# jinggqu/NextGen-UIA

Hardware: AMD Instinct MI355X
Metric: images/sec fwd+bwd BiomedCLIP+Mona bs=256 (higher is better)
Workload: dtype bf16

## Files before the change

### include/uia_hip.h

```cpp
#ifndef UIA_HIP_H
#define UIA_HIP_H
#include <stddef.h>
#include <stdint.h>

#ifdef __cplusplus
extern "C" {
#endif

enum { UIA_F32 = 0, UIA_BF16 = 1 };
enum { UIA_ACT_NONE = 0, UIA_ACT_GELU = 1, UIA_ACT_QUICKGELU = 2, UIA_ACT_RELU = 3 };
enum { UIA_MASK_NONE = 0, UIA_MASK_CAUSAL = 1, UIA_MASK_KEYPAD = 2 };
enum { UIA_MONA_BASELINE = 0, UIA_MONA_NOISE_AWARE = 1, UIA_MONA_FREQ_ENHANCED = 2, UIA_MONA_HYBRID = 3 };

const char* uia_last_error(void);
int uia_version(void);

typedef struct uia_gemm_desc {
    const void* A; int64_t lda;
    const void* W; int64_t ldw;
    int32_t M, N, K;
    float alpha;
    const float* bias;
    int32_t act;
    int32_t dact;
// ... 144 lines not shown
    const void* w1; const float* b1;
    const void* w2; const float* b2;
    float* y32;
    void* yT; int64_t yT_kb_rows;
    int64_t* rowsum_out;
    int32_t* ln_flag;
    void* u_out;
    void* t_out;
} uia_mona_fused_desc;
int uia_mona_fused_supported(int dtype, int D, int h, int w, int bott);
int uia_mona_fused_fwd(void* stream, int dtype, const uia_mona_fused_desc* d);

typedef struct uia_lora_rank_desc {
    int32_t M, N, nsrc;
    float alpha;
    const void* Q; int64_t ldq, q_stride;
    const void* W[3]; int64_t ldw;
    void* out; int64_t ldo;
    float drop_p;
    uint64_t seed[3];
} uia_lora_rank_desc;
int uia_lora_rank_update(void* stream, int dtype, const uia_lora_rank_desc* d);

typedef struct uia_ln_lora_desc {
    int32_t M, D, nsrc;
    float eps;
    const float* x; int64_t ldx;
    const float *gamma, *beta;
    void* h;
    const void* A[3]; int64_t lda;
    void* T; int64_t t_stride;
    float drop_p;
    uint64_t seed[3];
} uia_ln_lora_desc;
int uia_ln_lora_down(void* stream, int dtype, const uia_ln_lora_desc* d);

int uia_upsample_bilinear_fwd(void* stream, int B, int C, int h, int w, int H, int W, const float* src, int64_t ld, float* dst);
int uia_upsample_bilinear_bwd(void* stream, int B, int C, int h, int w, int H, int W, const float* ddst, float* dsrc, int64_t ld);
int uia_segment_mean_fwd(void* stream, int B, int n, int C, const float* x, int64_t ld, float* out);
int uia_segment_mean_bwd(void* stream, int B, int n, int C, const float* dout, float* dx, int64_t ld);
size_t uia_dicece_workspace_bytes(int B);
int uia_dicece_fwd_bwd(void* stream, int B, int C, int HW, const float* logits, const float* label, float smooth_nr, float smooth_dr,
                       float* ws, float* loss, float* dlogits);
size_t uia_focal_workspace_bytes(int N, int C);
int uia_focal_fwd_bwd(void* stream, int N, int C, const float* logits, const int64_t* labels, float gamma, float alpha, void* ws, size_t ws_bytes,
                      float* loss, float* dlogits);
size_t uia_binary_cls_stats_workspace_bytes(int N);
int uia_binary_cls_stats(void* stream, int N, const float* p1, const int64_t* labels, const int64_t* perm, void* ws, size_t ws_bytes, double* record);
size_t uia_surface_distances_workspace_bytes(int B, int H, int W);
int uia_surface_distances(void* stream, int B, int H, int W, const float* logits, const float* label, float percentile, void* ws, size_t ws_bytes,
                          double* hd, double* asd);
size_t uia_retrieval_workspace_bytes(int N, int E);
int uia_retrieval_ranks(void* stream, int N, int E, const float* img, const float* txt, int normalize, void* ws, size_t ws_bytes,
                        int32_t* gt_i2t, int32_t* eq_i2t, int32_t* gt_t2i, int32_t* eq_t2i);
size_t uia_retrieval_stats_workspace_bytes(int N);
int uia_retrieval_stats(void* stream, int N, const int32_t* gt, int nk, const int32_t* k_values, void* ws, size_t ws_bytes, double* record);

int uia_cast(void* stream, int dtype, size_t n, const float* src, void* dst, float scale);
int uia_transpose_cast(void* stream, int dtype, int rows, int cols, const float* src, void* dst);

typedef struct uia_pack_desc {
    const float* src;
    void* row;
    void* row_kb;
    void* tr;
    void* tr_kb;
    int32_t rows, cols;
    int32_t rows_pad, cols_pad;
    float scale;
    int32_t reserved_;
} uia_pack_desc;
int uia_pack_weights(void* stream, int dtype, int n, const uia_pack_desc* descs_device, int max_elems);
int uia_im2col(void* stream, int dtype, int B, int C, int H, int W, int P, const float* img, void* out);
int uia_im2col_padded(void* stream, int dtype, int B, int C, int H, int W, int P, const float* img, void* cols, int64_t ldo);
int uia_fill_cls(void* stream, int B, int N, int D, const float* cls, const float* pos0, float* x);
int uia_embed(void* stream, int rows, int L, int D, int vocab, int max_pos, const int64_t* ids, const float* table, const float* pos,
              const float* type0, float* out);
int uia_embed_packed(void* stream, int rows, int D, int vocab, int max_pos, const int64_t* ids, const int64_t* pos_idx, const float* table,
                     const float* pos, const float* type0, float* out);
int uia_embed_bwd(void* stream, int rows, int D, int vocab, const int64_t* ids, const float* dx, float* dtable, int64_t pad_id);
int uia_gather_rows(void* stream, int n, int D, const float* src, const int64_t* idx, float* dst);
int uia_copy_rows(void* stream, int rows, int64_t row_bytes, const void* src, int64_t src_stride_bytes, void* dst);
int uia_rows3_to_f32(void* stream, int rows, int D, int64_t stride_rows, const void* hi, int64_t ldhi, int64_t hi_kb_rows, const int8_t* lo, int64_t ldlo, float* dst);
int uia_dropout(void* stream, int dtype, size_t n, const void* src, void* dst, float p, uint64_t seed, int accumulate);
int uia_colsum(void* stream, int dtype, int M, int N, const void* A, int64_t lda, float* out);

int uia_layernorm_bwd_affine(void* stream, int dtype, int M, int D, const void* dy, const float* x, const float* gamma, float eps,
                             const float* dres, float* dx32, float* g_gamma, float* g_beta);
int uia_film_fwd(void* stream, int B, int N, int C, const float* x, const float* mul, const float* add, float* y);
int uia_film_bwd(void* stream, int B, int N, int C, const float* dy, const float* x, const float* mul, float* dx, float* dmul, float* dadd);
int uia_im2col3x3(void* stream, int dtype, int B, int h, int w, int C, int ntok, int tok_off, const float* x, void* cols);
int uia_col2im3x3(void* stream, int dtype, int B, int h, int w, int C, int ntok, int tok_off, const void* dcols, float* dx);
int uia_unshuffle(void* stream, int dtype, int B, int h, int w, int k1, int k2, const void* tmp, int64_t ld, float bias, float* out);
int uia_shuffle(void* stream, int dtype, int B, int h, int w, int k1, int k2, const float* dout, void* dtmp, int64_t ld);
int uia_act_bwd(void* stream, int dtype, size_t n, const void* dy, const void* y, int act, void* out);

size_t uia_infonce_workspace_bytes(int B, int E);
int uia_infonce_fwd_bwd(void* stream, int B, int E, const float* img, const float* txt, float inv_temp, float grad_scale,
                        float* loss, float* dimg, float* dtxt, void* workspace, size_t workspace_bytes);

int uia_adamw_clip_step(void* stream, size_t n, float* p, const float* g, float* m, float* v, float lr, float beta1, float beta2,
                        float eps, float weight_decay, float max_norm, int step, float grad_scale, float* ws2);

int uia_grad_accum_guarded(void* stream, size_t n, float* acc, float* mb, const float* loss, float* stats, int32_t* ctl, uint8_t* ok_log, int64_t log_index);
int uia_adamw_clip_step_guarded(void* stream, size_t n, float* p, float* acc, float* m, float* v, float lr, float lr_min, int t_max, float beta1, float beta2,
                                float eps, float weight_decay, float max_norm, float grad_scale, float skip_scale, float* ws8, int32_t* ctl);

enum { UIA_CONV3 = 0, UIA_CONVT_FWD = 1, UIA_CONVT_BWD = 2, UIA_CONV1 = 3 };
#define UIA_WGRAD_MAX_SPLITS 64
#define UIA_WGRAD_MAX_NARROW_SPLITS 512
#define UIA_WGRAD_MAX_DIRECT_SPLITS 1024
int uia_conv_igemm(void* stream, int dtype, int mode, int B, int H, int W, int C1, int C2, const void* x1, const void* x2, int N, int N1,
                   const void* w, const float* bias, void* y1, void* y2);
int uia_conv_wgrad_splits(int mode, int B, int H, int W, int C1, int C2, int N);
int uia_conv_igemm_form(int mode, int C1, int C2, int N, int N1);
int uia_conv_wgrad_form(int mode, int C1, int C2, int N);
int uia_conv_wgrad(void* stream, int dtype, int mode, int B, int H, int W, int C1, int C2, const void* x1, const void* x2, int N, const void* dy,
                   float* ws, float* dw);
#define UIA_BN_SLICES 256
int uia_bn_fwd(void* stream, int dtype, int training, int64_t M, int C, const void* y, const float* gamma, const float* beta, float* running_mean,
               float* running_var, int64_t* num_batches_tracked, float momentum, float eps, float* ws, float* mean, float* invstd, float* scale,
               float* shift, int relu, void* out);
int uia_bn_relu_bwd(void* stream, int dtype, int64_t M, int C, const void* y, const void* dout, const float* scale, const float* shift,
                    const float* mean, const float* invstd, const float* gamma, float* ws, float* dgamma, float* dbeta, void* dy);
int uia_colsum_ordered(void* stream, int dtype, int64_t M, int C, const void* y, float* ws, float* out);
int uia_bn_act_fwd(void* stream, int dtype, int training, int64_t M, int C, const void* y, const float* gamma, const float* beta, float* running_mean,
                   float* running_var, int64_t* num_batches_tracked, float momentum, float eps, float* ws, float* mean, float* invstd, float* scale,
                   float* shift, float slope, void* out, float drop_p, uint64_t seed, const uint8_t* keep_mask);
int uia_bn_act_bwd(void* stream, int dtype, int64_t M, int C, const void* y, const void* dout, const float* scale, const float* shift,
                   const float* mean, const float* invstd, const float* gamma, float* ws, float* dgamma, float* dbeta, void* dy, float slope,
                   float drop_p, uint64_t seed, const uint8_t* keep_mask);
int uia_maxpool2_fwd(void* stream, int dtype, int B, int H, int W, int C, const void* x, void* y);
int uia_maxpool2_bwd(void* stream, int dtype, int B, int H, int W, int C, const void* x, const void* dy, void* dx);
int uia_upsample_ac(void* stream, int dtype, int backward, int B, int H, int W, int C, int f, const void* in, void* out);
int uia_resize_aa(void* stream, int dtype, int backward, int B, int C, int Hi, int Wi, int Ho, int Wo, const void* x, float* tmp, float* out,
                  const float* dout, void* dx);

int uia_conv_strided(void* stream, int dtype, int dgrad, int B, int H, int W, int C, int k, int s, const void* x, int N, const void* w, void* y);
int uia_conv_strided_wgrad_splits(int B, int H, int W, int C, int k, int s, int N);
int uia_conv_strided_form(int dgrad, int C, int N, int k, int s);
int uia_conv_strided_wgrad_form(int C, int N, int k, int s);
int uia_conv_strided_wgrad(void* stream, int dtype, int B, int H, int W, int C, int k, int s, const void* x, int N, const void* dy, float* ws,
                           float* dw);
int uia_maxpool3s2_fwd(void* stream, int dtype, int B, int H, int W, int C, const void* x, void* y);
int uia_maxpool3s2_bwd(void* stream, int dtype, int B, int H, int W, int C, const void* x, const void* dy, void* dx);
int uia_bn_add_relu_fwd(void* stream, int dtype, int training, int64_t M, int C, const void* y, const void* r, const float* gamma, const float* beta,
                        float* running_mean, float* running_var, int64_t* num_batches_tracked, float momentum, float eps, float* ws, float* mean,
                        float* invstd, float* scale, float* shift, void* out);
int uia_bn_add_relu_bwd(void* stream, int dtype, int64_t M, int C, const void* y, const void* out, const void* dout, const float* mean,
                        const float* invstd, const float* gamma, float* ws, float* dgamma, float* dbeta, void* dy, void* dr);
int uia_avgpool_fwd(void* stream, int dtype, int B, int H, int W, int C, const void* x, float* pooled);
int uia_avgpool_bwd(void* stream, int dtype, int B, int H, int W, int C, const float* dout, void* dx);
int uia_nchw_to_nhwc(void* stream, int dtype, int B, int Cin, int H, int W, int Cout, int rep, const float* x, void* out);
int uia_add2(void* stream, int dtype, int64_t n, const void* a, const void* b, void* out);

int uia_comm_unique_id_bytes(void);
int uia_comm_get_unique_id(void* out, int bytes);
int uia_comm_init(int rank, int world, const void* unique_id, int bytes);
int uia_comm_world(void);
int uia_comm_initialised(void);
int uia_allreduce_sum(void* stream, int dtype, void* buf, size_t n);
int uia_allgather(void* stream, int dtype, const void* send, void* recv, size_t n_per_rank);
int uia_comm_destroy(void);

#ifdef __cplusplus
}
// ... 3 lines not shown
```

### nextgen-uia_amd/csrc/capi.cpp

```cpp
#include "uia_kernels.h"

void uia_set_error(const char* fmt, ...);
#define NEED(ptr, name) do { if (!(ptr)) { uia_set_error("%s: null descriptor", name); return -1; } } while (0)

extern "C" {

int uia_version(void) { return 100; }

int uia_gemm(void* stream, int dtype, const uia_gemm_desc* d, int tile_cfg) {
    NEED(d, "uia_gemm");
    return uia_gemm_launch((hipStream_t)stream, dtype, *d, tile_cfg);
}
int uia_lora_rank_update(void* stream, int dtype, const uia_lora_rank_desc* d) {
    NEED(d, "uia_lora_rank_update");
    return uia_lora_rank_update_launch((hipStream_t)stream, dtype, *d);
}
int uia_ln_lora_down(void* stream, int dtype, const uia_ln_lora_desc* d) {
    NEED(d, "uia_ln_lora_down");
    return uia_ln_lora_down_launch((hipStream_t)stream, dtype, *d);
}
int uia_wgrad(void* stream, int dtype, int M, int I, int J, const void* A, int64_t lda, const void* B, int64_t ldb, float alpha, float* dW, float* dbias_A) {
    return uia_wgrad_launch((hipStream_t)stream, dtype, M, I, J, A, lda, B, ldb, alpha, dW, dbias_A);
}
int uia_wgrad_ex(void* stream, int dtype, int M, int I, int J, const void* A, int64_t lda, const void* B, int64_t ldb, float alpha, float* dW, int64_t ldw,
                 int i_valid, int j_valid, float* dbias_A) {
    if (ldw <= 0) { uia_set_error("uia_wgrad_ex: ldw=%lld must be positive", (long long)ldw); return -1; }
    return uia_wgrad_launch((hipStream_t)stream, dtype, M, I, J, A, lda, B, ldb, alpha, dW, dbias_A, ldw, i_valid, j_valid);
}
int uia_wgrad_group(void* stream, int dtype, const uia_wgrad_group_desc* d) {
    if (!d) { uia_set_error("uia_wgrad_group: null descriptor"); return -1; }
    if (d->n < 1 || d->n > 4) { uia_set_error("uia_wgrad_group: n=%d outside 1..4", d->n); return -1; }
    if (d->ldw <= 0) { uia_set_error("uia_wgrad_group: ldw=%lld must be positive", (long long)d->ldw); return -1; }
    float* dW[4];
    float* db[4];
    for (int g = 0; g < 4; ++g) { dW[g] = d->dW[g]; db[g] = d->dbias_A[g]; }
    if (d->drop_p > 0.f) for (int g = 0; g < d->n; ++g) if (db[g]) { uia_set_error("uia_wgrad_group: dbias with dropout on B is not a form of the kernel"); return -1; }
    return uia_wgrad_group_launch((hipStream_t)stream, dtype, d->n, d->M, d->I, d->J, d->A, (long)d->lda, d->B, (long)d->ldb, d->alpha, dW, db, (long)d->ldw, d->i_valid, d->j_valid,
                                  d->drop_p, d->drop_seed, (long)d->drop_ld, d->drop_col0);
}
int uia_wgrad_drop(void* stream, int dtype, int M, int I, int J, const void* A, int64_t lda, const void* B, int64_t ldb, float alpha, float* dW, int64_t ldw,
                   int i_valid, int j_valid, float drop_p, uint64_t seed, int64_t drop_ld, int drop_col0) {
    if (ldw <= 0) { uia_set_error("uia_wgrad_drop: ldw=%lld must be positive", (long long)ldw); return -1; }
    if (!(drop_p > 0.f)) { uia_set_error("uia_wgrad_drop: drop_p=%f must be in (0, 1); uia_wgrad_ex is the form without dropout", (double)drop_p); return -1; }
    return uia_wgrad_launch((hipStream_t)stream, dtype, M, I, J, A, lda, B, ldb, alpha, dW, nullptr, ldw, i_valid, j_valid, drop_p, seed, drop_ld, drop_col0);
}
int uia_attn_fwd(void* stream, int dtype, const uia_attn_desc* d) {
    NEED(d, "uia_attn_fwd");
    return uia_attn_fwd_launch((hipStream_t)stream, dtype, *d);
}
int uia_attn_fwd_long(void* stream, int dtype, const uia_attn_desc* d) {
    NEED(d, "uia_attn_fwd_long");
    return uia_attn_fwd_long_launch((hipStream_t)stream, dtype, *d);
}
int uia_attn_bwd(void* stream, int dtype, const uia_attn_desc* d) {
    NEED(d, "uia_attn_bwd");
    return uia_attn_bwd_launch((hipStream_t)stream, dtype, *d, 0);
}
int uia_attn_bwd_cfg(void* stream, int dtype, const uia_attn_desc* d, int cfg) {
    NEED(d, "uia_attn_bwd_cfg");
    return uia_attn_bwd_launch((hipStream_t)stream, dtype, *d, cfg);
}
int uia_layernorm_fwd(void* stream, int dtype, int M, int D, int64_t ldx, const float* x, const float* gamma, const float* beta, float eps, void* yT, float* y32) {
    return uia_layernorm_fwd_launch((hipStream_t)stream, dtype, M, D, ldx, x, gamma, beta, eps, yT, y32, nullptr);
}
int uia_layernorm_fwd_stats(void* stream, int dtype, int M, int D, int64_t ldx, const float* x, const float* gamma, const float* beta, float eps, void* yT, float* y32,
                            float* stats) {
    return uia_layernorm_fwd_launch((hipStream_t)stream, dtype, M, D, ldx, x, gamma, beta, eps, yT, y32, stats);
}
int uia_layernorm_bwd(void* stream, int dtype, int M, int D, int64_t ldx, const void* dy, const float* x, const float* gamma, float eps, const float* dres, float* dx32, void* dxT) {
    return uia_layernorm_bwd_launch((hipStream_t)stream, dtype, M, D, ldx, dy, x, gamma, eps, dres, dx32, dxT);
}
int uia_layernorm_bwd3(void* stream, int dtype, int M, int D, int64_t ldx, const void* dy, const float* x, const void* x_hi, const int8_t* x_lo, int64_t x_kb_rows,
                       const float* gamma, float eps, const float* dres, const void* dres_hi, const int8_t* dres_lo, int64_t dres_kb_rows, float* dx32, void* dxT,
                       int8_t* dx_lo) {
    return uia_layernorm_bwd3_launch((hipStream_t)stream, dtype, M, D, ldx, dy, x, x_hi, x_lo, (long)x_kb_rows, gamma, eps, dres, dres_hi, dres_lo, (long)dres_kb_rows, dx32, dxT,
                                     dx_lo);
}
int uia_layernorm_bwd_periodic(void* stream, int dtype, int M, int D, const void* dy, const float* x, const void* x_hi, const int8_t* x_lo, int64_t x_kb_rows,
                               const float* gamma, float eps, const float* dres_rows, int period, float* dx32, void* dxT, int8_t* dx_lo) {
    return uia_layernorm_bwd_periodic_launch((hipStream_t)stream, dtype, M, D, dy, x, x_hi, x_lo, (long)x_kb_rows, gamma, eps, dres_rows, period, dx32, dxT, dx_lo);
}
int uia_attn_bwd_cls(void* stream, int dtype, const uia_attn_desc* d) {
    NEED(d, "uia_attn_bwd_cls");
    return uia_attn_bwd_cls_launch((hipStream_t)stream, dtype, *d);
}
int uia_attn_bwd_cls_rows(void* stream, int dtype, const uia_attn_desc* d) {
    NEED(d, "uia_attn_bwd_cls_rows");
    return uia_attn_bwd_cls_launch((hipStream_t)stream, dtype, *d, true);
}
int uia_attn_fwd_cls(void* stream, int dtype, const uia_attn_desc* d) {
    NEED(d, "uia_attn_fwd_cls");
    return uia_attn_fwd_cls_launch((hipStream_t)stream, dtype, *d);
}
int uia_mona_cls_fwd(void* stream, int dtype, int B, int ntok, const void* t, int64_t ldt, void* d, float p_drop, uint64_t seed, const uint8_t* keep_mask) {
    return uia_mona_cls_fwd_launch((hipStream_t)stream, dtype, B, ntok, t, (long)ldt, d, p_drop, seed, keep_mask);
}
int uia_rows3_to_f32(void* stream, int rows, int D, int64_t stride_rows, const void* hi, int64_t ldhi, int64_t hi_kb_rows, const int8_t* lo, int64_t ldlo, float* dst) {
    return uia_rows3_to_f32_launch((hipStream_t)stream, rows, D, (long)stride_rows, hi, (long)ldhi, (long)hi_kb_rows, lo, (long)ldlo, dst);
}
int uia_mona_cls_bwd(void* stream, int dtype, int B, int ntok, const void* dd, const void* t, int64_t ldt, void* dt, float p_drop, uint64_t seed, const uint8_t* keep_mask) {
    return uia_mona_cls_bwd_launch((hipStream_t)stream, dtype, B, ntok, dd, t, (long)ldt, dt, p_drop, seed, keep_mask);
}
int uia_copy_rows(void* stream, int rows, int64_t row_bytes, const void* src, int64_t src_stride_bytes, void* dst) {
    return uia_copy_rows_launch((hipStream_t)stream, rows, (long)row_bytes, src, (long)src_stride_bytes, dst);
}
int uia_cast(void* stream, int dtype, size_t n, const float* src, void* dst, float scale) { return uia_cast_launch((hipStream_t)stream, dtype, n, src, dst, scale); }
int uia_transpose_cast(void* stream, int dtype, int rows, int cols, const float* src, void* dst) { return uia_transpose_cast_launch((hipStream_t)stream, dtype, rows, cols, src, dst); }
int uia_pack_weights(void* stream, int dtype, int n, const uia_pack_desc* descs_device, int max_elems) { return uia_pack_weights_launch((hipStream_t)stream, dtype, n, descs_device, max_elems); }
int uia_im2col(void* stream, int dtype, int B, int C, int H, int W, int P, const float* img, void* out) { return uia_im2col_launch((hipStream_t)stream, dtype, B, C, H, W, P, img, out); }
int uia_fill_cls(void* stream, int B, int N, int D, const float* cls, const float* pos0, float* x) { return uia_fill_cls_launch((hipStream_t)stream, B, N, D, cls, pos0, x); }
int uia_embed(void* stream, int rows, int L, int D, int vocab, int max_pos, const int64_t* ids, const float* table, const float* pos, const float* type0, float* out) {
    return uia_embed_launch((hipStream_t)stream, rows, L, D, vocab, max_pos, ids, table, pos, type0, out);
}
int uia_gather_rows(void* stream, int n, int D, const float* src, const int64_t* idx, float* dst) { return uia_gather_rows_launch((hipStream_t)stream, n, D, src, idx, dst); }

int uia_mona_pre_fwd(void* stream, int dtype, int M, int D, const float* x, const float* norm_w, const float* norm_b, const float* gamma,
                     const float* gammax, float eps, void* u) {
    return uia_mona_pre_fwd_launch((hipStream_t)stream, dtype, M, D, x, norm_w, norm_b, gamma, gammax, eps, u);
}
int uia_mona_pre_bwd(void* stream, int dtype, int M, int D, const void* du, const float* x, const float* dy, const float* norm_w,
                     const float* norm_b, const float* gamma, const float* gammax, float eps, float* dx32, void* dxT, float* g_gamma,
                     float* g_gammax, float* g_norm_w, float* g_norm_b, float* ws, int64_t dxT_kb_rows) {
    return uia_mona_pre_bwd_launch((hipStream_t)stream, dtype, M, D, du, x, dy, norm_w, norm_b, gamma, gammax, eps, dx32, dxT, g_gamma, g_gammax,
                                   g_norm_w, g_norm_b, ws, (long)dxT_kb_rows);
}
int uia_mona_pre_fwd_t(void* stream, int dtype, int M, int D, const float* x, const float* norm_w, const float* norm_b, const float* gamma, const float* gammax,
                       float eps, void* u, const void* w1, int64_t ldw1, const float* b1, void* t, int64_t ldt) {
    return uia_mona_pre_fwd_t_launch((hipStream_t)stream, dtype, M, D, x, norm_w, norm_b, gamma, gammax, eps, u, w1, (long)ldw1, b1, t, (long)ldt);
}
int uia_mona_pre_bwd_du(void* stream, int dtype, int M, int D, const void* dt, int64_t ldt, const void* w1t, int64_t ldw1, const float* x, const float* dy,
                        const float* norm_w, const float* norm_b, const float* gamma, const float* gammax, float eps, float* dx32, void* dxT, float* g_gamma,
                        float* g_gammax, float* g_norm_w, float* g_norm_b, float* ws, int64_t dxT_kb_rows) {
    if (!dt || !w1t) { uia_set_error("uia_mona_pre_bwd_du: null dt / w1t"); return -1; }
    return uia_mona_pre_bwd_launch((hipStream_t)stream, dtype, M, D, nullptr, x, dy, norm_w, norm_b, gamma, gammax, eps, dx32, dxT, g_gamma, g_gammax,
                                   g_norm_w, g_norm_b, ws, (long)dxT_kb_rows, dt, (long)ldt, w1t, (long)ldw1);
}
int uia_mona_pre_bwd_du3(void* stream, int dtype, int M, int D, const void* dt, int64_t ldt, const void* w1t, int64_t ldw1, const float* x, const void* dy_hi, const int8_t* dy_lo,
                         const float* norm_w, const float* norm_b, const float* gamma, const float* gammax, float eps, void* dxT, int8_t* dx_lo, float* g_gamma,
                         float* g_gammax, float* g_norm_w, float* g_norm_b, float* ws, int64_t dxT_kb_rows) {
    if (!dt || !w1t || !dy_hi || !dy_lo || !dx_lo) { uia_set_error("uia_mona_pre_bwd_du3: null dt / w1t / dy_hi / dy_lo / dx_lo"); return -1; }
    return uia_mona_pre_bwd_launch((hipStream_t)stream, dtype, M, D, nullptr, x, nullptr, norm_w, norm_b, gamma, gammax, eps, nullptr, dxT, g_gamma, g_gammax,
                                   g_norm_w, g_norm_b, ws, (long)dxT_kb_rows, dt, (long)ldt, w1t, (long)ldw1, dy_hi, dy_lo, dx_lo);
}
size_t uia_mona_pre_bwd_workspace_bytes(int M, int D) { return uia_mona_pre_bwd_ws_floats(M, D) * sizeof(float); }
int uia_mona_spatial_fwd(void* stream, int dtype, const uia_mona_spatial_desc* d) {
    NEED(d, "uia_mona_spatial_fwd");
    return uia_mona_spatial_fwd_launch((hipStream_t)stream, dtype, *d);
}
int uia_mona_spatial_bwd(void* stream, int dtype, const uia_mona_spatial_desc* d) {
    NEED(d, "uia_mona_spatial_bwd");
    return uia_mona_spatial_bwd_launch((hipStream_t)stream, dtype, *d);
}
int uia_mona_fused_fwd(void* stream, int dtype, const uia_mona_fused_desc* d) {
    NEED(d, "uia_mona_fused_fwd");
    return uia_mona_fused_fwd_launch((hipStream_t)stream, dtype, *d);
}

size_t uia_infonce_workspace_bytes(int B, int E) { return uia_infonce_workspace_floats(B, E) * sizeof(float); }
int uia_infonce_fwd_bwd(void* stream, int B, int E, const float* img, const float* txt, float inv_temp, float grad_scale, float* loss,
                        float* dimg, float* dtxt, void* workspace, size_t workspace_bytes) {
    return uia_infonce_launch((hipStream_t)stream, B, E, img, txt, inv_temp, grad_scale, loss, dimg, dtxt, (float*)workspace, workspace_bytes / sizeof(float));
}
int uia_adamw_clip_step(void* stream, size_t n, float* p, const float* g, float* m, float* v, float lr, float beta1, float beta2, float eps,
                        float weight_decay, float max_norm, int step, float grad_scale, float* ws2) {
    return uia_adamw_clip_launch((hipStream_t)stream, n, p, g, m, v, lr, beta1, beta2, eps, weight_decay, max_norm, step, grad_scale, ws2);
}
int uia_grad_accum_guarded(void* stream, size_t n, float* acc, float* mb, const float* loss, float* stats, int32_t* ctl, uint8_t* ok_log, int64_t log_index) {
    return uia_grad_accum_guarded_launch((hipStream_t)stream, n, acc, mb, loss, stats, (int*)ctl, ok_log, (long)log_index);
}
int uia_adamw_clip_step_guarded(void* stream, size_t n, float* p, float* acc, float* m, float* v, float lr, float lr_min, int t_max, float beta1, float beta2,
                                float eps, float weight_decay, float max_norm, float grad_scale, float skip_scale, float* ws8, int32_t* ctl) {
    return uia_adamw_clip_guarded_launch((hipStream_t)stream, n, p, acc, m, v, lr, lr_min, t_max, beta1, beta2, eps, weight_decay, max_norm, grad_scale, skip_scale, ws8, (int*)ctl);
}

int uia_dropout(void* stream, int dtype, size_t n, const void* src, void* dst, float p, uint64_t seed, int accumulate) {
    return uia_dropout_launch((hipStream_t)stream, dtype, n, src, dst, p, seed, accumulate);
}
int uia_colsum(void* stream, int dtype, int M, int N, const void* A, int64_t lda, float* out) {
    return uia_colsum_launch((hipStream_t)stream, dtype, M, N, A, lda, out);
}

int uia_layernorm_bwd_affine(void* stream, int dtype, int M, int D, const void* dy, const float* x, const float* gamma, float eps, const float* dres,
                             float* dx32, float* g_gamma, float* g_beta) {
    return uia_layernorm_bwd_affine_launch((hipStream_t)stream, dtype, M, D, dy, x, gamma, eps, dres, dx32, g_gamma, g_beta);
}
int uia_film_fwd(void* stream, int B, int N, int C, const float* x, const float* mul, const float* add, float* y) { return uia_film_fwd_launch((hipStream_t)stream, B, N, C, x, mul, add, y); }
int uia_film_bwd(void* stream, int B, int N, int C, const float* dy, const float* x, const float* mul, float* dx, float* dmul, float* dadd) {
    return uia_film_bwd_launch((hipStream_t)stream, B, N, C, dy, x, mul, dx, dmul, dadd);
// ... 165 lines not shown
```

### nextgen-uia_amd/csrc/uia_kernels.h

```cpp
#pragma once
#include <hip/hip_runtime.h>
#include <stddef.h>
#include <stdint.h>

#include "../../include/uia_hip.h"

typedef uia_gemm_desc UiaGemmParams;
typedef uia_attn_desc UiaAttnParams;

int uia_gemm_launch(hipStream_t stream, int dtype, const UiaGemmParams& p, int cfg);
int uia_attn_fwd_launch(hipStream_t stream, int dtype, const UiaAttnParams& p);
int uia_attn_fwd_long_launch(hipStream_t stream, int dtype, const UiaAttnParams& p);
int uia_attn_bwd_launch(hipStream_t stream, int dtype, const UiaAttnParams& p, int cfg = 0);
int uia_layernorm_fwd_launch(hipStream_t stream, int dtype, int M, int D, long ldx, const float* x, const float* gamma, const float* beta,
                             float eps, void* yT, float* y32, float* stats);
int uia_layernorm_bwd_launch(hipStream_t stream, int dtype, int M, int D, long ldx, const void* dy, const float* x, const float* gamma, float eps,
                             const float* dres, float* dx32, void* dxT);
int uia_layernorm_bwd3_launch(hipStream_t stream, int dtype, int M, int D, long ldx, const void* dy, const float* x, const void* x_hi, const int8_t* x_lo,
                              long x_kb_rows, const float* gamma, float eps, const float* dres, const void* dres_hi, const int8_t* dres_lo, long dres_kb_rows,
                              float* dx32, void* dxT, int8_t* dx_lo);
int uia_layernorm_bwd_periodic_launch(hipStream_t stream, int dtype, int M, int D, const void* dy, const float* x, const void* x_hi, const int8_t* x_lo, long x_kb_rows,
                                      const float* gamma, float eps, const float* dres_rows, int period, float* dx32, void* dxT, int8_t* dx_lo);
int uia_attn_bwd_cls_launch(hipStream_t stream, int dtype, const UiaAttnParams& p, bool compact = false);
int uia_attn_fwd_cls_launch(hipStream_t stream, int dtype, const UiaAttnParams& p);
int uia_mona_cls_fwd_launch(hipStream_t stream, int dtype, int B, int ntok, const void* t, long ldt, void* d, float p_drop, uint64_t seed, const uint8_t* keep_mask);
int uia_rows3_to_f32_launch(hipStream_t stream, int rows, int D, long stride_rows, const void* hi, long ldhi, long hi_kb_rows, const int8_t* lo, long ldlo, float* dst);
int uia_mona_cls_bwd_launch(hipStream_t stream, int dtype, int B, int ntok, const void* dd, const void* t, long ldt, void* dt, float p_drop, uint64_t seed,
                            const uint8_t* keep_mask);
int uia_copy_rows_launch(hipStream_t stream, int rows, long row_bytes, const void* src, long src_stride_bytes, void* dst);
int uia_lora_rank_update_launch(hipStream_t stream, int dtype, const uia_lora_rank_desc& p);
int uia_ln_lora_down_launch(hipStream_t stream, int dtype, const uia_ln_lora_desc& p);
int uia_cast_launch(hipStream_t stream, int dtype, size_t n, const float* src, void* dst, float scale);
int uia_transpose_cast_launch(hipStream_t stream, int dtype, int rows, int cols, const float* src, void* dst);
int uia_pack_weights_launch(hipStream_t stream, int dtype, int n, const uia_pack_desc* descs_device, int max_elems);
int uia_im2col_launch(hipStream_t stream, int dtype, int B, int C, int H, int W, int P, const float* img, void* out);
int uia_fill_cls_launch(hipStream_t stream, int B, int N, int D, const float* cls, const float* pos0, float* x);
int uia_embed_launch(hipStream_t stream, int rows, int L, int D, int vocab, int max_pos, const int64_t* ids, const float* table, const float* pos, const float* type0, float* out);
int uia_gather_rows_launch(hipStream_t stream, int n, int D, const float* src, const int64_t* idx, float* dst);
int uia_wgrad_group_launch(hipStream_t stream, int dtype, int n, int M, int I, int J, const void* const* A, long lda, const void* const* B, long ldb, float alpha,
                            float* const* dW, float* const* dbias, long ldw, int i_valid, int j_valid, float drop_p, const uint64_t* drop_seed, long drop_ld, int drop_col0);
int uia_wgrad_launch(hipStream_t stream, int dtype, int M, int I, int J, const void* A, long lda, const void* B, long ldb, float alpha, float* dW, float* dbias,
                     long ldw = 0, int i_valid = 0, int j_valid = 0, float drop_p = 0.f, uint64_t drop_seed = 0, long drop_ld = 0, int drop_col0 = 0);
int uia_mona_pre_fwd_launch(hipStream_t stream, int dtype, int M, int D, const float* x, const float* nw, const float* nb, const float* gamma,
                            const float* gammax, float eps, void* u);
int uia_mona_pre_fwd_t_launch(hipStream_t stream, int dtype, int M, int D, const float* x, const float* nw, const float* nb, const float* gamma,
                              const float* gammax, float eps, void* u, const void* w1, long ldw1, const float* b1, void* t, long ldt);
int uia_mona_pre_bwd_launch(hipStream_t stream, int dtype, int M, int D, const void* du, const float* x, const float* dy, const float* nw,
                            const float* nb, const float* gamma, const float* gammax, float eps, float* dx32, void* dxT, float* g_gamma,
                            float* g_gammax, float* g_nw, float* g_nb, float* ws, long dxT_kb_rows, const void* dt = nullptr, long ldt = 0,
                            const void* w1t = nullptr, long ldw1 = 0, const void* dy_hi = nullptr, const int8_t* dy_lo = nullptr, int8_t* dx_lo = nullptr);
size_t uia_mona_pre_bwd_ws_floats(int M, int D);
int uia_mona_spatial_fwd_launch(hipStream_t stream, int dtype, const uia_mona_spatial_desc& p);
int uia_mona_spatial_bwd_launch(hipStream_t stream, int dtype, const uia_mona_spatial_desc& p);
int uia_mona_fused_fwd_launch(hipStream_t stream, int dtype, const uia_mona_fused_desc& q);
size_t uia_infonce_workspace_floats(int B, int E);
int uia_infonce_launch(hipStream_t stream, int B, int E, const float* img, const float* txt, float inv_temp, float grad_scale, float* loss,
                       float* dimg, float* dtxt, float* ws, size_t ws_floats);
int uia_adamw_clip_launch(hipStream_t stream, size_t n, float* p, const float* g, float* m, float* v, float lr, float beta1, float beta2,
                          float eps, float weight_decay, float max_norm, int step, float grad_scale, float* ws);
int uia_grad_accum_guarded_launch(hipStream_t stream, size_t n, float* acc, float* mb, const float* loss, float* stats, int* ctl, unsigned char* ok_log, long log_index);
int uia_adamw_clip_guarded_launch(hipStream_t stream, size_t n, float* p, float* acc, float* m, float* v, float lr, float lr_min, int t_max, float beta1,
                                  float beta2, float eps, float weight_decay, float max_norm, float grad_scale, float skip_scale, float* ws8, int* ctl);
int uia_dropout_launch(hipStream_t stream, int dtype, size_t n, const void* src, void* dst, float p, uint64_t seed, int accumulate);
int uia_colsum_launch(hipStream_t stream, int dtype, int M, int N, const void* A, long lda, float* out);
int uia_attn_small_launch(hipStream_t stream, int dtype, const UiaAttnParams& p, bool bwd);
bool uia_attn_dh16_ok(int dtype, const UiaAttnParams& p);
int uia_attn_dh16_launch(hipStream_t stream, const UiaAttnParams& p, bool bwd);
int uia_layernorm_bwd_affine_launch(hipStream_t stream, int dtype, int M, int D, const void* dy, const float* x, const float* gamma, float eps,
                                    const float* dres, float* dx32, float* g_gamma, float* g_beta);
int uia_film_fwd_launch(hipStream_t stream, int B, int N, int C, const float* x, const float* mul, const float* add, float* y);
int uia_film_bwd_launch(hipStream_t stream, int B, int N, int C, const float* dy, const float* x, const float* mul, float* dx, float* dmul, float* dadd);
int uia_im2col3x3_launch(hipStream_t stream, int dtype, int B, int h, int w, int C, int ntok, int tok_off, const float* x, void* cols);
int uia_col2im3x3_launch(hipStream_t stream, int dtype, int B, int h, int w, int C, int ntok, int tok_off, const void* dcols, float* dx);
int uia_unshuffle_launch(hipStream_t stream, int dtype, int B, int h, int w, int k1, int k2, const void* tmp, long ld, float bias, float* out);
int uia_shuffle_launch(hipStream_t stream, int dtype, int B, int h, int w, int k1, int k2, const float* dout, void* dtmp, long ld);
int uia_act_bwd_launch(hipStream_t stream, int dtype, size_t n, const void* dy, const void* y, int act, void* out);
size_t uia_mona_spatial_ws_floats(int B);
int uia_upsample_bilinear_launch(hipStream_t stream, bool bwd, int B, int C, int h, int w, int H, int W, const float* in, float* out, long ld);
int uia_segment_mean_launch(hipStream_t stream, bool bwd, int B, int n, int C, const float* in, float* out, long ld);
size_t uia_dicece_ws_floats(int B);
int uia_dicece_launch(hipStream_t stream, int B, int C, int HW, const float* logits, const float* label, float nr, float dr, float* ws, float* loss, float* dlogits);
size_t uia_focal_ws_bytes(int N, int C);
int uia_focal_launch(hipStream_t stream, int N, int C, const float* logits, const int64_t* labels, float gamma, float alpha, void* ws, size_t ws_bytes,
                     float* loss, float* dlogits);
size_t uia_binary_cls_stats_ws_bytes(int N);
int uia_binary_cls_stats_launch(hipStream_t stream, int N, const float* p1, const int64_t* labels, const int64_t* perm, void* ws, size_t ws_bytes,
                                double* record);
size_t uia_surface_ws_bytes(int B, int H, int W);
int uia_surface_launch(hipStream_t stream, int B, int H, int W, const float* logits, const float* label, float percentile, void* ws, size_t ws_bytes,
                       double* hd, double* asd);
size_t uia_retrieval_ranks_ws_bytes(int N, int E);
int uia_retrieval_ranks_launch(hipStream_t stream, int N, int E, const float* img, const float* txt, int normalize, void* ws, size_t ws_bytes,
                               int32_t* gt_i2t, int32_t* eq_i2t, int32_t* gt_t2i, int32_t* eq_t2i);
size_t uia_retrieval_stats_ws_bytes(int N);
int uia_retrieval_stats_launch(hipStream_t stream, int N, const int32_t* gt, int nk, const int32_t* k_values, void* ws, size_t ws_bytes, double* record);
int uia_im2col_padded_launch(hipStream_t stream, int dtype, int B, int C, int H, int W, int P, const float* img, void* out, long ldo);
int uia_embed_bwd_launch(hipStream_t stream, int rows, int D, int vocab, const int64_t* ids, const float* dx, float* dtable, long pad_id);
int uia_embed_packed_launch(hipStream_t stream, int rows, int D, int vocab, int max_pos, const int64_t* ids, const int64_t* pos_idx, const float* table, const float* pos, const float* type0, float* out);
int uia_ln_mean_rows_launch(hipStream_t stream, int B, int L, int row0, int n, int D, long ldx, const float* x, const float* gamma, const float* beta,
                            float eps, float* ws, float* out, long ldo);
int uia_conv_igemm_launch(hipStream_t stream, int dtype, int mode, int B, int H, int W, int C1, int C2, const void* x1, const void* x2, int N, int N1,
                          const void* w, const float* bias, void* y1, void* y2);
int uia_conv_wgrad_splits(int mode, int B, int H, int W, int C1, int C2, int N);
int uia_conv_wgrad_launch(hipStream_t stream, int dtype, int mode, int B, int H, int W, int C1, int C2, const void* x1, const void* x2, int N,
                          const void* dy, float* ws, float* dw);
int uia_bn_fwd_launch(hipStream_t stream, int dtype, int training, long M, int C, const void* y, const float* gamma, const float* beta,
                      float* run_mean, float* run_var, int64_t* nbt, float momentum, float eps, float* ws, float* mean, float* invstd,
                      float* scale, float* shift, int relu, void* out);
int uia_bn_relu_bwd_launch(hipStream_t stream, int dtype, long M, int C, const void* y, const void* dout, const float* scale, const float* shift,
                           const float* mean, const float* invstd, const float* gamma, float* ws, float* dgamma, float* dbeta, void* dy);
int uia_colsum_ordered_launch(hipStream_t stream, int dtype, long M, int C, const void* y, float* ws, float* out);
int uia_conv_igemm_form(int mode, int C1, int C2, int N, int N1);
// ... 28 lines not shown
```

### nextgen-uia_amd/uia_hip/_lib.py

```python
import ctypes as C
import os
import re

import torch

_HERE = os.path.dirname(os.path.abspath(__file__))
LIB_PATH = os.environ.get("UIA_HIP_LIB") or os.path.join(_HERE, "libuia_hip.so")

F32, BF16 = 0, 1
ACT_NONE, ACT_GELU, ACT_QUICKGELU, ACT_RELU = 0, 1, 2, 3
MASK_NONE, MASK_CAUSAL, MASK_KEYPAD = 0, 1, 2
MONA_VARIANTS = {"baseline": 0, "noise_aware": 1, "freq_enhanced": 2, "hybrid": 3}

vp, i32, i64, f32, sz = C.c_void_p, C.c_int32, C.c_int64, C.c_float, C.c_size_t


class PackDesc(C.Structure):
    _fields_ = [("src", vp), ("row", vp), ("row_kb", vp), ("tr", vp), ("tr_kb", vp), ("rows", i32), ("cols", i32),
                ("rows_pad", i32), ("cols_pad", i32), ("scale", f32), ("reserved_", i32)]


class GemmDesc(C.Structure):
    _fields_ = [("A", vp), ("lda", i64), ("W", vp), ("ldw", i64), ("M", i32), ("N", i32), ("K", i32), ("alpha", f32),
                ("bias", vp), ("act", i32), ("dact", i32), ("aux_in", vp), ("ldaux_in", i64), ("aux_out", vp), ("ldaux_out", i64),
                ("resid", vp), ("ldr", i64), ("resid_mod", i32), ("resid_row_off", i32), ("residT", vp), ("ldrT", i64),
                ("out_group", i32), ("outT", vp), ("ldo", i64), ("out32", vp), ("ldo32", i64), ("w_kblocked", i32),
                ("resid_ln_stats", vp), ("resid_ln_w", vp), ("resid_ln_b", vp),
                ("rowsum_out", vp), ("lnfold_sums", vp), ("lnfold_colsum", vp), ("lnfold_dim", i32), ("lnfold_eps", f32),
                ("resid_ln_dim", i32), ("resid_ln_eps", f32), ("a_kb_rows", i64), ("outT_kb_rows", i64), ("ln_flag", vp), ("ln_flag_limit", f32),
                ("drop_where", i32), ("drop_p", f32), ("drop_seed", C.c_uint64), ("a_drop_out", vp), ("splitk_ws", vp),
                ("A2", vp), ("lda2", i64), ("K2", i32), ("a2_group_cols", i32), ("a2_group_stride", i64),
                ("resid_lo8", vp), ("ld_resid_lo", i64), ("residT_kb_rows", i64), ("out_lo8", vp), ("ld_out_lo", i64),
                ("resid_lo_kb_rows", i64), ("out_lo_kb_rows", i64)]


class AttnDesc(C.Structure):
    _fields_ = [("q", vp), ("k", vp), ("v", vp), ("ld_qkv", i64), ("out", vp), ("ldo", i64), ("lse", vp), ("keylen", vp),
                ("B", i32), ("H", i32), ("L", i32), ("dh", i32), ("mask_kind", i32), ("scale", f32),
                ("dout", vp), ("lddo", i64), ("dq", vp), ("dk", vp), ("dv", vp), ("ld_dqkv", i64), ("cu_seqlens", vp),
                ("out_kb_rows", i64), ("dqkv_kb_rows", i64)]


class MonaSpatialDesc(C.Structure):
    _fields_ = [("variant", i32), ("B", i32), ("h", i32), ("w", i32), ("bott", i32),
                ("t", vp), ("d", vp),
                ("conv1_w", vp), ("conv1_b", vp), ("conv2_w", vp), ("conv2_b", vp), ("conv3_w", vp), ("conv3_b", vp),
                ("proj_w", vp), ("proj_b", vp), ("freq", vp), ("ne1_w", vp), ("ne1_b", vp), ("ne3_w", vp), ("ne3_b", vp),
                ("p_drop", f32), ("seed", C.c_uint64), ("keep_mask", vp),
                ("dd", vp), ("dt", vp),
                ("g_conv1_w", vp), ("g_conv1_b", vp), ("g_conv2_w", vp), ("g_conv2_b", vp), ("g_conv3_w", vp), ("g_conv3_b", vp),
                ("g_proj_w", vp), ("g_proj_b", vp), ("g_freq", vp), ("g_ne1_w", vp), ("g_ne1_b", vp), ("g_ne3_w", vp), ("g_ne3_b", vp), ("ws", vp)]


class WgradGroupDesc(C.Structure):
    _fields_ = [("n", C.c_int32), ("M", C.c_int32), ("I", C.c_int32), ("J", C.c_int32), ("A", C.c_void_p * 4), ("B", C.c_void_p * 4), ("dW", C.c_void_p * 4),
                ("dbias_A", C.c_void_p * 4), ("lda", C.c_int64), ("ldb", C.c_int64), ("ldw", C.c_int64), ("i_valid", C.c_int32), ("j_valid", C.c_int32),
                ("alpha", C.c_float), ("drop_p", C.c_float), ("drop_seed", C.c_uint64 * 4), ("drop_ld", C.c_int64), ("drop_col0", C.c_int32), ("reserved", C.c_int32)]


class LoraRankDesc(C.Structure):
    _fields_ = [("M", i32), ("N", i32), ("nsrc", i32), ("alpha", f32), ("Q", vp), ("ldq", i64), ("q_stride", i64), ("W", vp * 3), ("ldw", i64),
                ("out", vp), ("ldo", i64), ("drop_p", f32), ("seed", C.c_uint64 * 3)]


class LnLoraDesc(C.Structure):
    _fields_ = [("M", i32), ("D", i32), ("nsrc", i32), ("eps", f32), ("x", vp), ("ldx", i64), ("gamma", vp), ("beta", vp), ("h", vp), ("A", vp * 3), ("lda", i64),
                ("T", vp), ("t_stride", i64), ("drop_p", f32), ("seed", C.c_uint64 * 3)]


class MonaFusedDesc(C.Structure):
    _fields_ = [("sp", MonaSpatialDesc), ("D", i32), ("eps", f32), ("x", vp), ("norm_w", vp), ("norm_b", vp), ("gamma", vp), ("gammax", vp),
                ("w1", vp), ("b1", vp), ("w2", vp), ("b2", vp), ("y32", vp), ("yT", vp), ("yT_kb_rows", i64), ("rowsum_out", vp), ("ln_flag", vp),
                ("u_out", vp), ("t_out", vp)]


PROTOTYPES = {
    "uia_last_error": (C.c_char_p, []),
    "uia_version": (C.c_int, []),
    "uia_gemm": (C.c_int, [vp, C.c_int, C.POINTER(GemmDesc), C.c_int]),
    "uia_wgrad": (C.c_int, [vp, C.c_int, C.c_int, C.c_int, C.c_int, vp, i64, vp, i64, f32, vp, vp]),
    "uia_wgrad_drop": (C.c_int, [vp, C.c_int, C.c_int, C.c_int, C.c_int, vp, i64, vp, i64, f32, vp, i64, C.c_int, C.c_int, f32, C.c_uint64, i64, C.c_int]),
    "uia_wgrad_group": (C.c_int, [vp, C.c_int, vp]),
    "uia_wgrad_ex": (C.c_int, [vp, C.c_int, C.c_int, C.c_int, C.c_int, vp, i64, vp, i64, f32, vp, i64, C.c_int, C.c_int, vp]),
    "uia_attn_fwd": (C.c_int, [vp, C.c_int, C.POINTER(AttnDesc)]),
    "uia_attn_fwd_long": (C.c_int, [vp, C.c_int, C.POINTER(AttnDesc)]),
    "uia_attn_bwd": (C.c_int, [vp, C.c_int, C.POINTER(AttnDesc)]),
    "uia_attn_bwd_cfg": (C.c_int, [vp, C.c_int, C.POINTER(AttnDesc), C.c_int]),
    "uia_layernorm_fwd": (C.c_int, [vp, C.c_int, C.c_int, C.c_int, i64, vp, vp, vp, f32, vp, vp]),
    "uia_layernorm_fwd_stats": (C.c_int, [vp, C.c_int, C.c_int, C.c_int, i64, vp, vp, vp, f32, vp, vp, vp]),
    "uia_ln_mean_rows": (C.c_int, [vp, C.c_int, C.c_int, C.c_int, C.c_int, C.c_int, i64, vp, vp, vp, f32, vp, vp, i64]),
    "uia_conv_igemm": (C.c_int, [vp, C.c_int, C.c_int, C.c_int, C.c_int, C.c_int, C.c_int, C.c_int, vp, vp, C.c_int, C.c_int, vp, vp, vp, vp]),
    "uia_conv_wgrad_splits": (C.c_int, [C.c_int, C.c_int, C.c_int, C.c_int, C.c_int, C.c_int, C.c_int]),
    "uia_conv_wgrad": (C.c_int, [vp, C.c_int, C.c_int, C.c_int, C.c_int, C.c_int, C.c_int, C.c_int, vp, vp, C.c_int, vp, vp, vp]),
    "uia_conv_igemm_form": (C.c_int, [C.c_int, C.c_int, C.c_int, C.c_int, C.c_int]),
    "uia_conv_wgrad_form": (C.c_int, [C.c_int, C.c_int, C.c_int, C.c_int]),
    "uia_bn_act_fwd": (C.c_int, [vp, C.c_int, C.c_int, i64, C.c_int, vp, vp, vp, vp, vp, vp, f32, f32, vp, vp, vp, vp, vp, f32, vp, f32, C.c_uint64, vp]),
    "uia_bn_act_bwd": (C.c_int, [vp, C.c_int, i64, C.c_int, vp, vp, vp, vp, vp, vp, vp, vp, vp, vp, vp, f32, f32, C.c_uint64, vp]),
    "uia_maxpool2_fwd": (C.c_int, [vp, C.c_int, C.c_int, C.c_int, C.c_int, C.c_int, vp, vp]),
    "uia_maxpool2_bwd": (C.c_int, [vp, C.c_int, C.c_int, C.c_int, C.c_int, C.c_int, vp, vp, vp]),
    "uia_conv_strided": (C.c_int, [vp, C.c_int, C.c_int, C.c_int, C.c_int, C.c_int, C.c_int, C.c_int, C.c_int, vp, C.c_int, vp, vp]),
    "uia_conv_strided_wgrad_splits": (C.c_int, [C.c_int, C.c_int, C.c_int, C.c_int, C.c_int, C.c_int, C.c_int]),
    "uia_conv_strided_form": (C.c_int, [C.c_int, C.c_int, C.c_int, C.c_int, C.c_int]),
    "uia_conv_strided_wgrad_form": (C.c_int, [C.c_int, C.c_int, C.c_int, C.c_int]),
    "uia_conv_strided_wgrad": (C.c_int, [vp, C.c_int, C.c_int, C.c_int, C.c_int, C.c_int, C.c_int, C.c_int, vp, C.c_int, vp, vp, vp]),
    "uia_maxpool3s2_fwd": (C.c_int, [vp, C.c_int, C.c_int, C.c_int, C.c_int, C.c_int, vp, vp]),
    "uia_maxpool3s2_bwd": (C.c_int, [vp, C.c_int, C.c_int, C.c_int, C.c_int, C.c_int, vp, vp, vp]),
    "uia_bn_add_relu_fwd": (C.c_int, [vp, C.c_int, C.c_int, i64, C.c_int, vp, vp, vp, vp, vp, vp, vp, f32, f32, vp, vp, vp, vp, vp, vp]),
    "uia_bn_add_relu_bwd": (C.c_int, [vp, C.c_int, i64, C.c_int, vp, vp, vp, vp, vp, vp, vp, vp, vp, vp, vp]),
    "uia_avgpool_fwd": (C.c_int, [vp, C.c_int, C.c_int, C.c_int, C.c_int, C.c_int, vp, vp]),
    "uia_avgpool_bwd": (C.c_int, [vp, C.c_int, C.c_int, C.c_int, C.c_int, C.c_int, vp, vp]),
    "uia_nchw_to_nhwc": (C.c_int, [vp, C.c_int, C.c_int, C.c_int, C.c_int, C.c_int, C.c_int, C.c_int, vp, vp]),
    "uia_add2": (C.c_int, [vp, C.c_int, i64, vp, vp, vp]),
    "uia_bn_fwd": (C.c_int, [vp, C.c_int, C.c_int, i64, C.c_int, vp, vp, vp, vp, vp, vp, f32, f32, vp, vp, vp, vp, vp, C.c_int, vp]),
    "uia_bn_relu_bwd": (C.c_int, [vp, C.c_int, i64, C.c_int, vp, vp, vp, vp, vp, vp, vp, vp, vp, vp, vp]),
    "uia_colsum_ordered": (C.c_int, [vp, C.c_int, i64, C.c_int, vp, vp, vp]),
    "uia_upsample_ac": (C.c_int, [vp, C.c_int, C.c_int, C.c_int, C.c_int, C.c_int, C.c_int, C.c_int, vp, vp]),
    "uia_resize_aa": (C.c_int, [vp, C.c_int, C.c_int, C.c_int, C.c_int, C.c_int, C.c_int, C.c_int, C.c_int, vp, vp, vp, vp, vp]),
    "uia_layernorm_bwd": (C.c_int, [vp, C.c_int, C.c_int, C.c_int, i64, vp, vp, vp, f32, vp, vp, vp]),
    "uia_ln_lora_down": (C.c_int, [vp, C.c_int, C.POINTER(LnLoraDesc)]),
    "uia_lora_rank_update": (C.c_int, [vp, C.c_int, C.POINTER(LoraRankDesc)]),
    "uia_layernorm_bwd3": (C.c_int, [vp, C.c_int, C.c_int, C.c_int, i64, vp, vp, vp, vp, i64, vp, f32, vp, vp, vp, i64, vp, vp, vp]),
    "uia_mona_pre_fwd": (C.c_int, [vp, C.c_int, C.c_int, C.c_int, vp, vp, vp, vp, vp, f32, vp]),
    "uia_mona_pre_bwd": (C.c_int, [vp, C.c_int, C.c_int, C.c_int, vp, vp, vp, vp, vp, vp, vp, f32, vp, vp, vp, vp, vp, vp, vp, i64]),
    "uia_mona_pre_fwd_t": (C.c_int, [vp, C.c_int, C.c_int, C.c_int, vp, vp, vp, vp, vp, f32, vp, vp, i64, vp, vp, i64]),
    "uia_mona_pre_bwd_du": (C.c_int, [vp, C.c_int, C.c_int, C.c_int, vp, i64, vp, i64, vp, vp, vp, vp, vp, vp, f32, vp, vp, vp, vp, vp, vp, vp, i64]),
    "uia_mona_pre_bwd_du3": (C.c_int, [vp, C.c_int, C.c_int, C.c_int, vp, i64, vp, i64, vp, vp, vp, vp, vp, vp, vp, f32, vp, vp, vp, vp, vp, vp, vp, i64]),
    "uia_mona_pre_bwd_workspace_bytes": (sz, [C.c_int, C.c_int]),
    "uia_mona_spatial_fwd": (C.c_int, [vp, C.c_int, C.POINTER(MonaSpatialDesc)]),
    "uia_mona_spatial_bwd": (C.c_int, [vp, C.c_int, C.POINTER(MonaSpatialDesc)]),
    "uia_mona_spatial_workspace_bytes": (sz, [C.c_int]),
    "uia_mona_fused_supported": (C.c_int, [C.c_int, C.c_int, C.c_int, C.c_int, C.c_int]),
    "uia_mona_fused_fwd": (C.c_int, [vp, C.c_int, C.POINTER(MonaFusedDesc)]),
    "uia_upsample_bilinear_fwd": (C.c_int, [vp, C.c_int, C.c_int, C.c_int, C.c_int, C.c_int, C.c_int, vp, C.c_int64, vp]),
    "uia_upsample_bilinear_bwd": (C.c_int, [vp, C.c_int, C.c_int, C.c_int, C.c_int, C.c_int, C.c_int, vp, vp, C.c_int64]),
    "uia_segment_mean_fwd": (C.c_int, [vp, C.c_int, C.c_int, C.c_int, vp, C.c_int64, vp]),
    "uia_segment_mean_bwd": (C.c_int, [vp, C.c_int, C.c_int, C.c_int, vp, vp, C.c_int64]),
    "uia_dicece_workspace_bytes": (sz, [C.c_int]),
    "uia_dicece_fwd_bwd": (C.c_int, [vp, C.c_int, C.c_int, C.c_int, vp, vp, C.c_float, C.c_float, vp, vp, vp]),
    "uia_focal_workspace_bytes": (sz, [C.c_int, C.c_int]),
    "uia_focal_fwd_bwd": (C.c_int, [vp, C.c_int, C.c_int, vp, vp, f32, f32, vp, sz, vp, vp]),
    "uia_binary_cls_stats_workspace_bytes": (sz, [C.c_int]),
    "uia_binary_cls_stats": (C.c_int, [vp, C.c_int, vp, vp, vp, vp, sz, vp]),
    "uia_surface_distances_workspace_bytes": (sz, [C.c_int, C.c_int, C.c_int]),
    "uia_surface_distances": (C.c_int, [vp, C.c_int, C.c_int, C.c_int, vp, vp, f32, vp, sz, vp, vp]),
    "uia_retrieval_workspace_bytes": (sz, [C.c_int, C.c_int]),
    "uia_retrieval_ranks": (C.c_int, [vp, C.c_int, C.c_int, vp, vp, C.c_int, vp, sz, vp, vp, vp, vp]),
    "uia_retrieval_stats_workspace_bytes": (sz, [C.c_int]),
    "uia_retrieval_stats": (C.c_int, [vp, C.c_int, vp, C.c_int, vp, vp, sz, vp]),
    "uia_infonce_workspace_bytes": (sz, [C.c_int, C.c_int]),
    "uia_infonce_fwd_bwd": (C.c_int, [vp, C.c_int, C.c_int, vp, vp, f32, f32, vp, vp, vp, vp, sz]),
    "uia_adamw_clip_step": (C.c_int, [vp, sz, vp, vp, vp, vp, f32, f32, f32, f32, f32, f32, C.c_int, f32, vp]),
    "uia_grad_accum_guarded": (C.c_int, [vp, sz, vp, vp, vp, vp, vp, vp, i64]),
    "uia_adamw_clip_step_guarded": (C.c_int, [vp, sz, vp, vp, vp, vp, f32, f32, C.c_int, f32, f32, f32, f32, f32, f32, f32, vp, vp]),
    "uia_comm_unique_id_bytes": (C.c_int, []),
    "uia_comm_get_unique_id": (C.c_int, [vp, C.c_int]),
    "uia_comm_init": (C.c_int, [C.c_int, C.c_int, vp, C.c_int]),
    "uia_comm_world": (C.c_int, []),
    "uia_comm_initialised": (C.c_int, []),
    "uia_allreduce_sum": (C.c_int, [vp, C.c_int, vp, sz]),
    "uia_allgather": (C.c_int, [vp, C.c_int, vp, vp, sz]),
    "uia_comm_destroy": (C.c_int, []),
    "uia_dropout": (C.c_int, [vp, C.c_int, sz, vp, vp, f32, C.c_uint64, C.c_int]),
    "uia_colsum": (C.c_int, [vp, C.c_int, C.c_int, C.c_int, vp, i64, vp]),
    "uia_layernorm_bwd_affine": (C.c_int, [vp, C.c_int, C.c_int, C.c_int, vp, vp, vp, f32, vp, vp, vp, vp]),
    "uia_film_fwd": (C.c_int, [vp, C.c_int, C.c_int, C.c_int, vp, vp, vp, vp]),
    "uia_film_bwd": (C.c_int, [vp, C.c_int, C.c_int, C.c_int, vp, vp, vp, vp, vp, vp]),
    "uia_im2col3x3": (C.c_int, [vp, C.c_int, C.c_int, C.c_int, C.c_int, C.c_int, C.c_int, C.c_int, vp, vp]),
    "uia_col2im3x3": (C.c_int, [vp, C.c_int, C.c_int, C.c_int, C.c_int, C.c_int, C.c_int, C.c_int, vp, vp]),
    "uia_unshuffle": (C.c_int, [vp, C.c_int, C.c_int, C.c_int, C.c_int, C.c_int, C.c_int, vp, i64, f32, vp]),
    "uia_shuffle": (C.c_int, [vp, C.c_int, C.c_int, C.c_int, C.c_int, C.c_int, C.c_int, vp, vp, i64]),
    "uia_act_bwd": (C.c_int, [vp, C.c_int, sz, vp, vp, C.c_int, vp]),
    "uia_cast": (C.c_int, [vp, C.c_int, sz, vp, vp, f32]),
    "uia_transpose_cast": (C.c_int, [vp, C.c_int, C.c_int, C.c_int, vp, vp]),
    "uia_pack_weights": (C.c_int, [vp, C.c_int, C.c_int, vp, C.c_int]),
    "uia_im2col": (C.c_int, [vp, C.c_int, C.c_int, C.c_int, C.c_int, C.c_int, C.c_int, vp, vp]),
    "uia_im2col_padded": (C.c_int, [vp, C.c_int, C.c_int, C.c_int, C.c_int, C.c_int, C.c_int, vp, vp, C.c_int64]),
    "uia_fill_cls": (C.c_int, [vp, C.c_int, C.c_int, C.c_int, vp, vp, vp]),
    "uia_embed": (C.c_int, [vp, C.c_int, C.c_int, C.c_int, C.c_int, C.c_int, vp, vp, vp, vp, vp]),
    "uia_embed_bwd": (C.c_int, [vp, C.c_int, C.c_int, C.c_int, vp, vp, vp, C.c_int64]),
    "uia_embed_packed": (C.c_int, [vp, C.c_int, C.c_int, C.c_int, C.c_int, vp, vp, vp, vp, vp, vp]),
    "uia_gather_rows": (C.c_int, [vp, C.c_int, C.c_int, vp, vp, vp]),
    "uia_copy_rows": (C.c_int, [vp, C.c_int, i64, vp, i64, vp]),
    "uia_attn_bwd_cls": (C.c_int, [vp, C.c_int, C.POINTER(AttnDesc)]),
    "uia_mona_cls_bwd": (C.c_int, [vp, C.c_int, C.c_int, C.c_int, vp, vp, i64, vp, f32, C.c_uint64, vp]),
    "uia_attn_fwd_cls": (C.c_int, [vp, C.c_int, C.POINTER(AttnDesc)]),
    "uia_attn_bwd_cls_rows": (C.c_int, [vp, C.c_int, C.POINTER(AttnDesc)]),
    "uia_mona_cls_fwd": (C.c_int, [vp, C.c_int, C.c_int, C.c_int, vp, i64, vp, f32, C.c_uint64, vp]),
    "uia_rows3_to_f32": (C.c_int, [vp, C.c_int, C.c_int, i64, vp, i64, i64, vp, i64, vp]),
    "uia_layernorm_bwd_periodic": (C.c_int, [vp, C.c_int, C.c_int, C.c_int, vp, vp, vp, vp, i64, vp, f32, vp, C.c_int, vp, vp, vp]),
}

_lib = None
_BLOCKING = ("uia_comm_init", "uia_comm_destroy", "uia_comm_get_unique_id")


class UiaError(RuntimeError):
    pass


def lib():
    global _lib
    if _lib is None:
        if not os.path.exists(LIB_PATH):
            raise UiaError(f"{LIB_PATH} not built: run `make -C nextgen-uia_amd/csrc` (hipcc --offload-arch=gfx950). "
                           "There is no CPU fallback for the uia hot path.")
        release = os.environ.get("UIA_CTYPES_RELEASE_GIL", "0") == "1"
        handle = (C.CDLL if release else C.PyDLL)(LIB_PATH)
        blocking = C.CDLL(LIB_PATH)
        _one_copy_of("librccl")
        _one_copy_of("libamdhip64")
        for name, (res, args) in PROTOTYPES.items():
            fn = getattr(blocking if name in _BLOCKING else handle, name)
            fn.restype, fn.argtypes = res, args
            if name in _BLOCKING:
                setattr(handle, name, fn)
        _lib = handle
    return _lib


def _one_copy_of(stem):
    try:
        pat = re.compile(r"^" + re.escape(stem) + r"\.so(\.\d+)*$")
        paths = {line.split()[-1] for line in open("/proc/self/maps") if pat.match(os.path.basename(line.split()[-1]) if line.split() else "")}
    except OSError:
        return
    real = {os.path.realpath(p) for p in paths}
    if len(real) > 1:
        raise UiaError(f"two copies of {stem} are loaded ({sorted(real)}): import torch before uia_hip so that libuia_hip.so binds to PyTorch's runtime")


def check(rc, what=""):
    if rc != 0:
        raise UiaError(f"{what} failed (rc={rc}): {lib().uia_last_error().decode()}")
```

### nextgen-uia_amd/uia_hip/functional.py

```python
import math
import os
import weakref

import time

import torch

from . import handoff, ops
from ._lib import UiaError
from .handoff import (ClsGrad, Resid3, _g3_partner_feeds, cls_grad_of, fwd3_of, grad3_decode, grad3_of, grad_resid3_enabled, hook_free, linear_chain,
                      publish_cls_grad, publish_fwd3, publish_grad3, publish_rows, publish_t_copy, set_cls_grad, set_grad_resid3, t_copy_of, take_rows, zero_sums,
                      cls_only, set_cls_forward, take_cls_forward)
from .handoff import clear as clear_t_copies

_STATE = {"dtype": torch.bfloat16, "seed": 0x5EED, "calls": 0, "fwd_resid3": os.environ.get("UIA_FWD_RESID3", "1") != "0"}


def set_compute_dtype(dt):
    assert dt in (torch.bfloat16, torch.float32)
    _STATE["dtype"] = dt


def compute_dtype():
    return _STATE["dtype"]
# ... 141 lines not shown
        self._table = None

    def _refreshed(self, items):
        ready = ops.Ready()
        for it in items:
            it.fwd.refreshed(ready)
            it.bwd.refreshed(ready)
            for view, _, _, _ in it.extra:
                ext = self._ext_of.get(view.untyped_storage().data_ptr())
                ext = ext() if ext is not None else None
                if ext is not None:
                    ext.ready = ready

    def _repack(self, items):
        dt, dev = items[0].dt, items[0].row.device
        entries = [e for it in items for e in it.entries()]
        table, n, mx = ops.pack_table(entries, dev)
        ops.pack_weights(table, n, mx, dt)
        for it in items:
            it.version, it.epoch, it.src_ptr = it.ref()._version, self.epoch, it.ref().data_ptr()
        self._refreshed(items)
        return table, n, mx, dt, entries

    def bump(self):
        self.epoch += 1
        if len(self._c) > 8192:
            alive = lambda r: all(x() is not None for x in r) if isinstance(r, tuple) else r() is not None
            self._c = {k: v for k, v in self._c.items() if alive(v[1])}
        live = [it for it in self._packed.values() if it.ref() is not None]
        if len(live) != len(self._packed):
            self._packed = {id(it.ref()): it for it in live}
            self._table = None
        if not live:
            return
        groups = {}
        for it in live:
            groups.setdefault((it.dt, it.row.device), []).append(it)
        tables = self._table if isinstance(self._table, dict) else {}
        fresh = {}
        for key, items in groups.items():
            sig = (sum(1 + len(it.extra) for it in items), tuple(id(it) for it in items))
            hit = tables.get(key)
            if hit is not None and hit[5] == sig and all(it.src_ptr == it.ref().data_ptr() for it in items):
                table, n, mx, dt, _, _ = hit
                ops.pack_weights(table, n, mx, dt)
                for it in items:
                    it.version, it.epoch = it.ref()._version, self.epoch
                self._refreshed(items)
                fresh[key] = hit
            else:
                fresh[key] = self._repack(items) + (sig,)
        self._table = fresh

    def _packed_get(self, p, dt, transpose, pads=None):
        it = self._packed.get(id(p))
        want = tuple(pads) if pads is not None else tuple(p.shape)
        if it is None or it.ref() is not p or it.dt != dt or it.row.device != p.device or tuple(it.row.shape) != want or it.pads != pads:
            old = it
            it = _PackedParam(p, dt, pads)
            if old is not None and old.ref() is p and old.dt == dt and old.row.device == p.device:
                it.extra = [e for e in old.extra if (self._ext_of.get(e[0].untyped_storage().data_ptr()) or (lambda: None))() is not None]
            self._packed[id(p)] = it
            self._table = None
        if it.version != p._version or it.epoch != self.epoch:
            self._repack([it])
        return it.bwd if transpose else it.fwd

    def get_lnfold(self, w, b, ln_w, ln_b, dt):
        key = (id(w), id(ln_w), dt, "lnfold")
        vers = (w._version, ln_w._version, ln_b._version, -1 if b is None else b._version, w.device)
        hit = self._c.get(key)
        if hit is not None and hit[0] == vers and hit[1]() is w and hit[3]() is ln_w:
            return hit[2]
        with torch.no_grad():
            w32 = w.detach().float()
            wf = (w32 * ln_w.detach().float()[None, :]).to(dt).contiguous()
            colsum = wf.float().sum(1).contiguous()
            bias = (w32 @ ln_b.detach().float())
            if b is not None:
                bias = bias + b.detach().float()
            bias = bias.contiguous()
        out = (ops.PackedW(wf), colsum, bias)
        self._c[key] = (vers, weakref.ref(w), out, weakref.ref(ln_w))
        return out

    def get_cat(self, ws, dt, transpose=False):
        key = (tuple(id(w) for w in ws), dt, transpose, "cat")
        vers = tuple(w._version for w in ws)
        hit = self._c.get(key)
        if hit is not None and hit[0] == vers and all(r() is w for r, w in zip(hit[1], ws)) and hit[2].device == ws[0].device:
            return hit[2]
        with torch.no_grad():
            cat = torch.cat([w.detach().float() for w in ws], 0)
            src = cat.t().contiguous() if transpose else cat
            out = ops.PackedW(src.to(dt).contiguous())
        self._c[key] = (vers, tuple(weakref.ref(w) for w in ws), out)
        return out

    def get_lora_ext(self, ws, Bs, scaling, dt, rp=64):
        key = (tuple(id(w) for w in ws), tuple(id(b) for b in Bs), dt, float(scaling), "ext")
        vers = tuple(w._version for w in ws)
        hit = self._c.get(key)
        pads = [(b.shape[0], max(rp, b.shape[1])) for b in Bs]
        if hit is not None and hit[0] == vers and all(r() is t for r, t in zip(hit[1], tuple(ws) + tuple(Bs))) and hit[2].device == ws[0].device:
            for b, pd in zip(Bs, pads):
                self._packed_get(b, dt, False, pd)
            return hit[2]
        g = 64 // torch.empty(0, dtype=dt).element_size()
        Ntot, K = sum(w.shape[0] for w in ws), ws[0].shape[1]
        assert K % g == 0 and rp % g == 0 and all(w.shape[1] == K for w in ws) and all(b.shape[0] == w.shape[0] for b, w in zip(Bs, ws))
        with torch.no_grad():
            kb = torch.zeros((K + rp) // g, Ntot, g, device=ws[0].device, dtype=dt)
            kb[:K // g] = torch.cat([w.detach().float() for w in ws], 0).to(dt).view(Ntot, K // g, g).permute(1, 0, 2)
        off = 0
        for b, pd in zip(Bs, pads):
            self._packed_get(b, dt, False, pd)
            it = self._packed[id(b)]
            it.extra = [e for e in it.extra if e[0].untyped_storage().data_ptr() != kb.untyped_storage().data_ptr()]
            it.extra.append((kb[K // g:, off:off + b.shape[0], :], Ntot, rp, float(scaling)))
            self._table = None
            self._repack([it])
            off += b.shape[0]
        out = ops.ExtW(kb, Ntot, K + rp, rp)
        self._ext_of = {k: r for k, r in self._ext_of.items() if r() is not None}
        self._ext_of[kb.untyped_storage().data_ptr()] = weakref.ref(out)
        self._c[key] = (vers, tuple(weakref.ref(t) for t in tuple(ws) + tuple(Bs)), out)
        return out

    def get(self, p, dt, transpose=False, pad_rows_to=None, pad_cols_to=None):
        padded = pad_rows_to is not None or pad_cols_to is not None
        if (p.requires_grad and (dt != torch.float32 or padded) and p.dim() == 2 and p.is_cuda
                and p.dtype == torch.float32 and p.is_contiguous() and 0 < p.numel() <= self.PACK_MAX_ELEMS):
            pads = (max(p.shape[0], pad_rows_to or 0), max(p.shape[1], pad_cols_to or 0)) if padded else None
            return self._packed_get(p, dt, transpose, pads)
        key = (id(p), dt, transpose, pad_rows_to, pad_cols_to)
        hit = self._c.get(key)
        if hit is not None and hit[0] == p._version and hit[1]() is p and hit[2].device == p.device and (not p.requires_grad or hit[3] == self.epoch):
            return hit[2]
        src = p.detach()
        if src.dim() != 2:
            src = src.reshape(src.shape[0], -1)
        src = src.contiguous().float()
        if pad_rows_to is not None and src.shape[0] < pad_rows_to:
            src = torch.cat([src, src.new_zeros(pad_rows_to - src.shape[0], src.shape[1])], 0)
        if pad_cols_to is not None and src.shape[1] < pad_cols_to:
            src = torch.cat([src, src.new_zeros(src.shape[0], pad_cols_to - src.shape[1])], 1)
        if transpose:
            out = torch.empty(src.shape[1], src.shape[0], device=src.device, dtype=dt)
            ops.transpose_cast(src, out)
        elif dt == torch.float32:
            out = src
        else:
            out = torch.empty(src.shape, device=src.device, dtype=dt)
            ops.cast(src, out)
        out = ops.PackedW(out)
        self._c[key] = (p._version, weakref.ref(p), out, self.epoch)
        return out


WEIGHTS = WeightCache()


def _empty(shape, dt, like):
    return torch.empty(shape, device=like.device, dtype=dt)


# ... 168 lines not shown
        G = ({k: p.grad for k, p in zip(names, ctx.direct_params)} if direct
             else {k: torch.zeros_like(v, dtype=torch.float32) for k, v in P.items()})
        w2t = WEIGHTS.get(P["project2.weight"], dt, transpose=True)
        dd = _empty((M, bott), dt, x)
        side = _wgrad_side_stream(x.device) if _STATE.get("wgrad_side_stream", False) else None
        _wgrad_beside(side, lambda: ops.gemm(dy_t, w2t, out_t=dd), dy_t, d, G["project2.weight"], G["project2.bias"])
        sp = {_SPATIAL_MAP[k]: v.detach().contiguous() for k, v in P.items() if k in _SPATIAL_MAP}
        sg = {_SPATIAL_MAP[k]: G[k] for k in P if k in _SPATIAL_MAP}
        dtt = _empty((M, bott), dt, x)
        ops.mona_spatial_bwd(variant, B, h, w, t, sp, dd, dtt, sg, p_drop=p_drop, seed=seed, keep_mask=keep_mask)
        w1t = WEIGHTS.get(P["project1.weight"], dt, transpose=True)
        du = None if fuse_du else _empty((M, D), dt, x)
        _wgrad_beside(side, None if fuse_du else (lambda: ops.gemm(dtt, w1t, out_t=du)), dtt, u, G["project1.weight"], G["project1.bias"])
        need_dx = ctx.needs_input_grad[0]
        dx_t = _act(M, D, dt, x, 4 * D) if (need_dx and dt != torch.float32) else None
        w1t_rows = (dtt, w1t.row if isinstance(w1t, ops.PackedW) else w1t) if fuse_du else None
        if need_dx and g3 is not None and fuse_du and getattr(ctx, "g3_out", False):
            dlo = torch.empty(M, D, device=x.device, dtype=torch.int8)
            ops.mona_pre_bwd(None, x, g3, P["norm.weight"], P["norm.bias"], P["gamma"], P["gammax"], None, dx_t,
                             G["gamma"], G["gammax"], G["norm.weight"], G["norm.bias"], dt_w1t=w1t_rows, dx_lo=dlo)
            dx = publish_grad3(x.shape, x.device, dx_t, dlo)
        else:
            if need_dx and g3 is not None:
                dy = g3.decode().view(B, N, D)
            dx = torch.empty_like(x) if need_dx else None
            ops.mona_pre_bwd(du, x, dy if need_dx else None, P["norm.weight"], P["norm.bias"], P["gamma"], P["gammax"], dx, dx_t,
                             G["gamma"], G["gammax"], G["norm.weight"], G["norm.bias"], dt_w1t=w1t_rows)
            if need_dx:
                publish_t_copy(dx, dx_t)
        grads = tuple(None if direct else (G[k] if ctx.needs_input_grad[7 + i] else None) for i, k in enumerate(names))
        return (dx, None, None, None, None, None, None) + grads


def _wgrad_beside(side, dgrad, a, b, dw, db):
    if side is not None:
        side.wait_stream(torch.cuda.current_stream())
        with torch.cuda.stream(side):
            ops.wgrad(a, b, dw, db)
        a.record_stream(side)
        b.record_stream(side)
    if dgrad is not None:
        dgrad()
    if side is None:
        ops.wgrad(a, b, dw, db)


_WGRAD_SIDE = {}


def _wgrad_side_stream(device):
    key = device.index if device.index is not None else torch.cuda.current_device()
    if key not in _WGRAD_SIDE:
        _WGRAD_SIDE[key] = torch.cuda.Stream(device=device)
    return _WGRAD_SIDE[key]


def set_wgrad_side_stream(flag):
    _STATE["wgrad_side_stream"] = bool(flag)


def join_side_streams():
    cur = torch.cuda.current_stream()
    for st in _WGRAD_SIDE.values():
        cur.wait_stream(st)


DIRECT_TRAIN = True


def _is_flat_grad(p):
    g = p.grad
    return (getattr(p, "_uia_flat_grad", False) and g is not None and g.dtype == torch.float32 and g.is_contiguous() and g.shape == p.shape
            and g.device == p.device)


def mona_apply(x_bnd, module_params, variant, hw, p_drop, training, keep_mask=None):
    names = tuple(k for k in MONA_PARAM_ORDER if k in module_params)
    pd = p_drop if (training or keep_mask is not None) else 0.0
    params = [module_params[k] for k in names]
    direct = torch.is_grad_enabled() and all(p.requires_grad and _is_flat_grad(p) for p in params)
    return MonaFn.apply(x_bnd, variant, tuple(hw), pd, keep_mask, names, direct, *params)


class BlockSpec:

    def __init__(self, heads, eps, act, ln1, qkv, proj, ln2, fc1, fc2, mask=None, publish_out=False):
        self.heads, self.eps, self.act, self.mask = heads, eps, act, mask
        self.publish_out = publish_out
        self.ln1, self.qkv, self.proj, self.ln2, self.fc1, self.fc2 = ln1, qkv, proj, ln2, fc1, fc2


ATTN_SINGLE_PASS_MAX = 272


class VitBlockFn(torch.autograd.Function):

    @staticmethod
    def forward(ctx, x, spec):
        B, N, D = x.shape
        M, dt = B * N, compute_dtype()
        if N > ATTN_SINGLE_PASS_MAX and (ctx.needs_input_grad[0] or spec.mask is not None):
            raise UiaError(f"vit_block: {N} tokens exceed the {ATTN_SINGLE_PASS_MAX} of the attention backward; sequences this long run forward-only "
                           "(frozen tower under torch.no_grad()), unmasked" if ctx.needs_input_grad[0] else
                           f"vit_block: {N} tokens with a mask: the long attention forward takes no mask")
        x3 = fwd3_of(x)
        like = x3.lo if x3 is not None else x
        if x3 is None:
            x = x.contiguous()
            x2d = x.view(M, D)
        train = ctx.needs_input_grad[0]
        fold = ln_fold_enabled(dt, M)
        if x3 is not None:
            assert fold and dt == torch.bfloat16, "a three-byte forward token reached a block that cannot take it"
            rows = (x3.hi, x3.sums)
        else:
            rows = take_rows(x, dt) if fold else None
        qkv = _empty((M, 3 * D), dt, like)
        if rows is not None:
            wq, cq, bq = WEIGHTS.get_lnfold(spec.qkv[0], spec.qkv[1], spec.ln1[0], spec.ln1[1], dt)
            xin_t, sums0 = rows
            if not ops.is_kb(xin_t):
                xin_t = xin_t.view(M, D)
            ops.gemm(xin_t, wq, bias=bq, out_t=qkv, lnfold=(sums0, cq, D, spec.eps))
            h1 = _act(M, D, dt, like, spec.fc1[0].shape[0]) if x3 is not None else xin_t
        else:
            h1 = _empty((M, D), dt, x)
            ops.layernorm_fwd(x2d, spec.ln1[0], spec.ln1[1], spec.eps, y_t=h1)
            ops.gemm(h1, WEIGHTS.get(spec.qkv[0], dt), bias=spec.qkv[1], out_t=qkv)
        if handoff.take_last_block_cls() and spec.mask is None and 1 < N <= ATTN_SINGLE_PASS_MAX and D == 64 * spec.heads and like.is_cuda:
            return VitBlockFn._forward_cls(ctx, x, x3, qkv, spec, (B, N, D), dt, train)
        if N > ATTN_SINGLE_PASS_MAX:
            a = _empty((M, D), dt, like)
            ops.attn_fwd_long(qkv[:, :D], qkv[:, D:2 * D], qkv[:, 2 * D:], a, B, spec.heads, N)
            lse = None
        else:
            a = _attn_act(M, D, dt, like, D) if D == 64 * spec.heads else _empty((M, D), dt, like)
            lse = torch.empty(B, spec.heads, N, device=like.device, dtype=torch.float32) if train else None
            ops.attn_fwd(qkv[:, :D], qkv[:, D:2 * D], qkv[:, 2 * D:], a, B, spec.heads, N, lse=lse, mask=spec.mask)
        F = spec.fc1[0].shape[0]
        f = _act(M, F, dt, like, D)
        pre = _empty((M, F), dt, like) if train else None
        r3 = fold and _STATE.get("block_resid3", False) and dt == torch.bfloat16 and M > 2048
        x1 = None if r3 else torch.empty(M, D, device=like.device, dtype=torch.float32)
        lo1 = torch.empty(M, D, device=like.device, dtype=torch.int8) if r3 else None
        if fold:
            sums1 = zero_sums(M, like.device)
            h1 = _as_act(h1, M, D, dt, F) if x3 is None else h1
            resx = dict(resid3=x3.resid3) if x3 is not None else dict(resid=x2d)
            ops.gemm(a, WEIGHTS.get(spec.proj[0], dt), bias=spec.proj[1], out32=x1, out_t=h1, out_lo=lo1, rowsum=sums1, **resx)
            w1, c1, b1 = WEIGHTS.get_lnfold(spec.fc1[0], spec.fc1[1], spec.ln2[0], spec.ln2[1], dt)
            ops.gemm(h1, w1, bias=b1, act=spec.act, aux_out=pre, out_t=f, lnfold=(sums1, c1, D, spec.eps))
        else:
            ops.gemm(a, WEIGHTS.get(spec.proj[0], dt), bias=spec.proj[1], resid=x2d, out32=x1)
            h1 = _as_act(h1, M, D, dt, 0)
            ops.layernorm_fwd(x1, spec.ln2[0], spec.ln2[1], spec.eps, y_t=h1)
            ops.gemm(h1, WEIGHTS.get(spec.fc1[0], dt), bias=spec.fc1[1], act=spec.act, aux_out=pre, out_t=f)
        x2 = torch.empty(B, N, D, device=like.device, dtype=torch.float32)
        res1 = dict(resid3=Resid3(h1, lo1)) if r3 else dict(resid=x1)
        if fold and spec.publish_out:
            sums2 = zero_sums(M, like.device)
            h2 = _act(M, D, dt, like, 3 * D) if r3 else _as_act(h1, M, D, dt, 3 * D)
            ops.gemm(f, WEIGHTS.get(spec.fc2[0], dt), bias=spec.fc2[1], out32=x2.view(M, D), out_t=h2, rowsum=sums2, **res1)
            publish_rows(x2, h2, sums2)
        else:
            ops.gemm(f, WEIGHTS.get(spec.fc2[0], dt), bias=spec.fc2[1], out32=x2.view(M, D), **res1)
        if train:
            saved, ctx.layout = handoff.save_layout(x3.resid3 if x3 is not None else x, qkv, a, lse, Resid3(h1, lo1) if r3 else x1, pre)
            ctx.save_for_backward(*saved)
            ctx.xshape = (B, N, D)
            ctx.spec = spec
            ctx.g3_out = dt == torch.bfloat16 and _g3_partner_feeds(x)
            ctx.cls_ok = spec.mask is None and N <= ATTN_SINGLE_PASS_MAX and D == 64 * spec.heads and not r3 and handoff.cls_grad_enabled()
        return x2

    @staticmethod
    def _forward_cls(ctx, x, x3, qkv, spec, shape, dt, train):
        B, N, D = shape
        like = qkv
        a = _empty((B, D), dt, like)
        lse = torch.empty(B, spec.heads, device=like.device, dtype=torch.float32) if train else None
        ops.attn_fwd_cls(qkv[:, :D], qkv[:, D:2 * D], qkv[:, 2 * D:], a, B, spec.heads, N, lse=lse)
        x_cls = torch.empty(B, D, device=like.device, dtype=torch.float32)
        if x3 is not None:
            ops.rows3_to_f32(x3.hi, x3.lo, N, x_cls)
        else:
            ops.copy_rows(x.view(B * N, D), N, x_cls)
        x1 = torch.empty(B, D, device=like.device, dtype=torch.float32)
        M = B * N
        wp = WEIGHTS.get(spec.proj[0], dt)
        ops.gemm(a, wp, bias=spec.proj[1], resid=x_cls, out32=x1, tile_cfg=_rows_tile_cfg(M, wp, like, dt, out32=True, resid=True))
        h2 = _empty((B, D), dt, like)
        ops.layernorm_fwd(x1, spec.ln2[0], spec.ln2[1], spec.eps, y_t=h2)
        F = spec.fc1[0].shape[0]
        f = _empty((B, F), dt, like)
        pre = _empty((B, F), dt, like) if train else None
        w1, w2 = WEIGHTS.get(spec.fc1[0], dt), WEIGHTS.get(spec.fc2[0], dt)
        ops.gemm(h2, w1, bias=spec.fc1[1], act=spec.act, aux_out=pre, out_t=f, tile_cfg=_rows_tile_cfg(M, w1, like, dt, act=True, aux_out=train, out_t=True))
        x2 = torch.empty(B, 1, D, device=like.device, dtype=torch.float32)
        ops.gemm(f, w2, bias=spec.fc2[1], resid=x1, out32=x2.view(B, D), tile_cfg=_rows_tile_cfg(M, w2, like, dt, out32=True, resid=True))
        if train:
            saved, ctx.layout = handoff.save_layout(x3.resid3 if x3 is not None else x, qkv, a, lse, x1, pre)
            ctx.save_for_backward(*saved)
            ctx.xshape = (B, N, D)
            ctx.spec = spec
            ctx.g3_out = dt == torch.bfloat16 and _g3_partner_feeds(x)
            ctx.cls_ok = False
            ctx.cls_fwd = True
        handoff.cls_rows_out(True)
        return x2

    @staticmethod
    def backward_cls(ctx, cg):
        compact = getattr(ctx, "cls_fwd", False)
        xin, qkv, a, lse, x1, pre = handoff.restore_layout(ctx.saved_tensors, ctx.layout)
        x3_in = isinstance(xin, Resid3)
        x = xin.lo if x3_in else xin
        spec = ctx.spec
        B, N, D = ctx.xshape
        M, dt = B * N, qkv.dtype
        F = pre.shape[1]
        dy = cg.rows32
        dy_t = dy if dt == torch.float32 else (cg.rows_t if cg.rows_t is not None else t_copy_of(dy, dt))
        pre_cls = pre if compact else ops.copy_rows(pre, N, _empty((B, F), dt, x))
        dpre = _empty((B, F), dt, x)
        ops.gemm(dy_t, WEIGHTS.get(spec.fc2[0], dt, transpose=True), dact=spec.act, aux_in=pre_cls, out_t=dpre)
        dh = _empty((B, D), dt, x)
        ops.gemm(dpre, WEIGHTS.get(spec.fc1[0], dt, transpose=True), out_t=dh)
        x1_cls = x1 if compact else ops.copy_rows(x1, N, _empty((B, D), torch.float32, x))
        dx1 = _empty((B, D), torch.float32, x)
        dx1_t = _empty((B, D), dt, x) if dt != torch.float32 else dx1
        ops.layernorm_bwd(dh, x1_cls, spec.ln2[0], spec.eps, dres=dy, dx32=dx1, dx_t=dx1_t if dt != torch.float32 else None)
        da = dh
        ops.gemm(dx1_t, WEIGHTS.get(spec.proj[0], dt, transpose=True), out_t=da)
        dqkv = _attn_act(M, 3 * D, dt, x, D)
        if ops.is_kb(dqkv):
            ops.attn_bwd_cls(qkv[:, :D], qkv[:, D:2 * D], qkv[:, 2 * D:], a, da, lse, dqkv, None, None, B, spec.heads, N, rows=compact)
        else:
            ops.attn_bwd_cls(qkv[:, :D], qkv[:, D:2 * D], qkv[:, 2 * D:], a, da, lse, dqkv[:, :D], dqkv[:, D:2 * D], dqkv[:, 2 * D:], B, spec.heads, N, rows=compact)
        dh1 = _empty((M, D), dt, x)
        ops.gemm(dqkv, WEIGHTS.get(spec.qkv[0], dt, transpose=True), out_t=dh1)
        xrows = xin if x3_in else x.view(M, D)
        if getattr(ctx, "g3_out", False):
            dx_t = _empty((M, D), dt, x)
            dlo = torch.empty(M, D, device=x.device, dtype=torch.int8)
            ops.layernorm_bwd_periodic(dh1, xrows, spec.ln1[0], spec.eps, dx1, N, dx_t=dx_t, dx_lo=dlo)
            return publish_grad3((B, N, D), x.device, dx_t, dlo), None
        dx = torch.empty(B, N, D, device=x.device, dtype=torch.float32)
        if dt == torch.float32:
            ops.layernorm_bwd_periodic(dh1, xrows, spec.ln1[0], spec.eps, dx1, N, dx32=dx.view(M, D))
            return dx, None
        dx_t = _empty((M, D), dt, x)
        ops.layernorm_bwd(dh1, xrows, spec.ln1[0], spec.eps, dres=ClsGrad(dx1, None, N).decode().view(M, D), dx32=dx.view(M, D), dx_t=dx_t)
        publish_t_copy(dx, dx_t)
        return dx, None

    @staticmethod
    def backward(ctx, dx2):
        if getattr(ctx, "cls_fwd", False):
            dx2 = dx2.contiguous()
            B, N, D = ctx.xshape
            dt = ctx.saved_tensors[-1].dtype
            return VitBlockFn.backward_cls(ctx, ClsGrad(dx2.view(B, D), t_copy_of(dx2, dt).view(B, D) if dt != torch.float32 else None, N))
        cg = cls_grad_of(dx2)
        if cg is not None:
            if getattr(ctx, "cls_ok", False):
                return VitBlockFn.backward_cls(ctx, cg)
            dx2 = cg.decode()
        g3 = grad3_of(dx2)
        xin, qkv, a, lse, x1, pre = handoff.restore_layout(ctx.saved_tensors, ctx.layout)
        x3_in, r3 = isinstance(xin, Resid3), isinstance(x1, Resid3)
        x = xin.lo if x3_in else xin
        spec = ctx.spec
        B, N, D = ctx.xshape
        M, dt = B * N, qkv.dtype
        F = pre.shape[1]
        if g3 is not None:
            dx2_t = g3.hi if ops.is_kb(g3.hi) else g3.hi.view(M, D)
            dres2 = Resid3(dx2_t, g3.lo)
        else:
            dx2 = dx2.contiguous()
            dx2_t = t_copy_of(dx2, dt, allow_kb=True)
            if not ops.is_kb(dx2_t):
                dx2_t = dx2_t.view(M, D)
            dres2 = dx2.view(M, D)
        g3_mode = g3 is not None or getattr(ctx, "g3_out", False)
        dpre = _act(M, F, dt, x, D)
        ops.gemm(dx2_t, WEIGHTS.get(spec.fc2[0], dt, transpose=True), dact=spec.act, aux_in=pre, out_t=dpre)
        dh = _empty((M, D), dt, x)
        ops.gemm(dpre, WEIGHTS.get(spec.fc1[0], dt, transpose=True), out_t=dh)
        del dpre
        if r3 or g3_mode:
            dx1_t = _empty((M, D), dt, x)
            dlo1 = torch.empty(M, D, device=x.device, dtype=torch.int8)
            ops.layernorm_bwd(dh, x1, spec.ln2[0], spec.eps, dres=dres2, dx_t=dx1_t, dx_lo=dlo1)
            dx1 = Resid3(dx1_t, dlo1)
        else:
            dx1 = torch.empty_like(x1)
            dx1_t = _empty((M, D), dt, x) if dt != torch.float32 else dx1
            ops.layernorm_bwd(dh, x1, spec.ln2[0], spec.eps, dres=dres2, dx32=dx1, dx_t=dx1_t if dt != torch.float32 else None)
        da = dh
        ops.gemm(dx1_t, WEIGHTS.get(spec.proj[0], dt, transpose=True), out_t=da)
        dqkv = _attn_act(M, 3 * D, dt, x, D) if D == 64 * spec.heads else _empty((M, 3 * D), dt, x)
        if ops.is_kb(dqkv):
            ops.attn_bwd(qkv[:, :D], qkv[:, D:2 * D], qkv[:, 2 * D:], a, da, lse, dqkv, None, None, B, spec.heads, N, mask=spec.mask)
        else:
            ops.attn_bwd(qkv[:, :D], qkv[:, D:2 * D], qkv[:, 2 * D:], a, da, lse, dqkv[:, :D], dqkv[:, D:2 * D], dqkv[:, 2 * D:], B, spec.heads, N, mask=spec.mask)
        ops.gemm(dqkv, WEIGHTS.get(spec.qkv[0], dt, transpose=True), out_t=da)
        dx_t = _empty((M, D), dt, x) if dt != torch.float32 else None
        xrows = xin if x3_in else x.view(M, D)
        if getattr(ctx, "g3_out", False):
            dlo = torch.empty(M, D, device=x.device, dtype=torch.int8)
            ops.layernorm_bwd(da, xrows, spec.ln1[0], spec.eps, dres=dx1, dx_t=dx_t, dx_lo=dlo)
            return publish_grad3((B, N, D), x.device, dx_t, dlo), None
        dx = torch.empty(B, N, D, device=x.device, dtype=torch.float32)
        ops.layernorm_bwd(da, xrows, spec.ln1[0], spec.eps, dres=dx1, dx32=dx.view(M, D), dx_t=dx_t)
        publish_t_copy(dx, dx_t)
        return dx, None


def vit_block(x, spec):
    return VitBlockFn.apply(x, spec)


class LnResidual:
    __slots__ = ("raw", "stats", "w", "b", "dim", "eps", "hi", "lo")

    def __init__(self, raw, stats, w, b, dim=None, eps=None, hi=None, lo=None):
        self.raw, self.stats, self.w, self.b = raw, stats, w, b
        self.dim, self.eps = dim, eps
        self.hi, self.lo = hi, lo

    def gemm_kw(self):
        if self.lo is not None:
            return dict(resid3=Resid3(self.hi, self.lo), resid_ln=(self.stats, self.w, self.b, self.dim, self.eps))
        if self.stats is None:
            return dict(resid=self.raw)
        if self.dim is None:
            return dict(resid=self.raw, resid_ln=(self.stats, self.w, self.b))
        return dict(resid=self.raw, resid_ln=(self.stats, self.w, self.b, self.dim, self.eps))


def _post_ln(raw, w, b, eps, x_t, stats_buf=None):
    if _STATE.get("text_ln_deferred", True):
        stats = stats_buf if stats_buf is not None else torch.empty(raw.shape[0], 2, device=raw.device, dtype=torch.float32)
        ops.layernorm_fwd(raw, w, b, eps, y_t=x_t, stats=stats)
        return LnResidual(raw, stats, w, b)
    ops.layernorm_fwd(raw, w, b, eps, y_t=x_t, y32=raw)
    return LnResidual(raw, None, w, b)


def post_ln_embed(e32, ln, x_t):
    return _post_ln(e32, ln.weight, ln.bias, ln.eps, x_t)


def _res_cls_rows(res, L, B, D, eps):
    rows = torch.empty(B, D, device=res.w.device, dtype=torch.float32)
    if res.lo is not None:
        ops.rows3_to_f32(res.hi, res.lo, L, rows)
    else:
        ops.copy_rows(res.raw.view(-1, D), L, rows)
        if res.stats is None:
            return rows
    ops.layernorm_fwd(rows, res.w, res.b, res.eps if res.eps is not None else eps, y32=rows)
    return rows


def post_ln_layer_cls_ok(x_t, heads, L, cu_seqlens=None):
    D = x_t.cols if ops.is_kb(x_t) else x_t.shape[1]
    return cu_seqlens is None and D == 64 * heads and 1 < L <= 288 and x_t.is_cuda and not (x_t.dtype != torch.float32 and _STATE.get("text_resid_t", False))


def _post_ln_layer_cls(res, qkv, L, B, heads, P, keylen, eps, D, dt):
    a = _empty((B, D), dt, qkv)
    ops.attn_fwd_cls(qkv[:, :D], qkv[:, D:2 * D], qkv[:, 2 * D:], a, B, heads, L, mask="keypad", keylen=keylen)
    r = _res_cls_rows(res, L, B, D, eps)
    s_a = torch.empty(B, D, device=qkv.device, dtype=torch.float32)
    M = B * L
    wo = WEIGHTS.get(P["attention.output.dense.weight"], dt)
    ops.gemm(a, wo, bias=P["attention.output.dense.bias"], resid=r, out32=s_a, tile_cfg=_rows_tile_cfg(M, wo, qkv, dt, out32=True, resid=True))
    h = _empty((B, D), dt, qkv)
    ops.layernorm_fwd(s_a, P["attention.output.LayerNorm.weight"], P["attention.output.LayerNorm.bias"], eps, y_t=h, y32=s_a)
    F = P["intermediate.dense.weight"].shape[0]
    f = _empty((B, F), dt, qkv)
    w1, w2 = WEIGHTS.get(P["intermediate.dense.weight"], dt), WEIGHTS.get(P["output.dense.weight"], dt)
    ops.gemm(h, w1, bias=P["intermediate.dense.bias"], act="gelu", out_t=f, tile_cfg=_rows_tile_cfg(M, w1, qkv, dt, act=True, out_t=True))
    ops.gemm(f, w2, bias=P["output.dense.bias"], resid=s_a, out32=r, tile_cfg=_rows_tile_cfg(M, w2, qkv, dt, out32=True, resid=True))
    ops.layernorm_fwd(r, P["output.LayerNorm.weight"], P["output.LayerNorm.bias"], eps, y_t=h, y32=r)
    return LnResidual(r, None, P["output.LayerNorm.weight"], P["output.LayerNorm.bias"]), h


def post_ln_layer(res, x_t, L, B, heads, P, keylen, eps=1e-12, cu_seqlens=None, fold_sums=None, fold_out=False, cls_only=False):
    kb_in = ops.is_kb(x_t)
    M, D = (x_t.rows, x_t.cols) if kb_in else x_t.shape
    dt = x_t.dtype
    t_resid = dt != torch.float32 and _STATE.get("text_resid_t", False)
    fold = fold_sums is not None and ln_fold_enabled(dt, M) and not t_resid
    qkv = _empty((M, 3 * D), dt, x_t)
    if res.dim is not None:
        wq, cq, bq = WEIGHTS.get_lnfold(P["_qkv_raw"][0], P["_qkv_raw"][1], res.w, res.b, dt)
        ops.gemm(x_t, wq, bias=bq, out_t=qkv, lnfold=(res.stats, cq, D, res.eps))
    else:
        ops.gemm(x_t, P["_qkv_w"](dt), bias=P["_qkv_b"], out_t=qkv)
    if cls_only:
        return _post_ln_layer_cls(res, qkv, L, B, heads, P, keylen, eps, D, dt)
    a = _attn_act(M, D, dt, x_t, D) if (D == 64 * heads and cu_seqlens is None) else _empty((M, D), dt, x_t)
    if cu_seqlens is not None:
        ops.attn_fwd(qkv[:, :D], qkv[:, D:2 * D], qkv[:, 2 * D:], a, B, heads, L, cu_seqlens=cu_seqlens)
    else:
        ops.attn_fwd(qkv[:, :D], qkv[:, D:2 * D], qkv[:, 2 * D:], a, B, heads, L, mask="keypad", keylen=keylen)
    del qkv
    F = P["intermediate.dense.weight"].shape[0]
    f = _act(M, F, dt, x_t, D)
    r3 = fold and _STATE.get("text_resid3", True) and dt == torch.bfloat16 and M > 2048
    if fold:
        lw_a, lb_a = P["attention.output.LayerNorm.weight"], P["attention.output.LayerNorm.bias"]
        s_a_t = _act(M, D, dt, x_t, F)
        if r3:
            lo_a = torch.empty(M, D, device=x_t.device, dtype=torch.int8)
            ops.gemm(a, WEIGHTS.get(P["attention.output.dense.weight"], dt), bias=P["attention.output.dense.bias"], out_t=s_a_t, out_lo=lo_a,
                     rowsum=fold_sums[0], **res.gemm_kw())
            res_a = LnResidual(None, fold_sums[0], lw_a, lb_a, D, eps, hi=s_a_t, lo=lo_a)
        else:
            s_a = torch.empty(M, D, device=x_t.device, dtype=torch.float32)
            ops.gemm(a, WEIGHTS.get(P["attention.output.dense.weight"], dt), bias=P["attention.output.dense.bias"], out32=s_a, out_t=s_a_t,
                     rowsum=fold_sums[0], **res.gemm_kw())
            res_a = LnResidual(s_a, fold_sums[0], lw_a, lb_a, D, eps)
        w1, c1, b1 = WEIGHTS.get_lnfold(P["intermediate.dense.weight"], P["intermediate.dense.bias"], lw_a, lb_a, dt)
        ops.gemm(s_a_t, w1, bias=b1, act="gelu", out_t=f, lnfold=(fold_sums[0], c1, D, eps))
        if not r3:
            del s_a_t
    else:
        s_a = torch.empty(M, D, device=x_t.device, dtype=torch.float32)
        ops.gemm(a, WEIGHTS.get(P["attention.output.dense.weight"], dt), bias=P["attention.output.dense.bias"], out32=s_a,
                 **(dict(resid_t=x_t) if t_resid else res.gemm_kw()))
        x_t = _as_act(x_t, M, D, dt, 0)
        res_a = _post_ln(s_a, P["attention.output.LayerNorm.weight"], P["attention.output.LayerNorm.bias"], eps, x_t)
        ops.gemm(x_t, WEIGHTS.get(P["intermediate.dense.weight"], dt), bias=P["intermediate.dense.bias"], act="gelu", out_t=f)
    s_o = res.raw if res.raw is not None else torch.empty(M, D, device=x_t.device, dtype=torch.float32)
    if fold and fold_out:
        x_t = _as_act(x_t, M, D, dt, 3 * D)
        if r3:
            lo_o = res.lo if res.lo is not None else torch.empty(M, D, device=x_t.device, dtype=torch.int8)
            ops.gemm(f, WEIGHTS.get(P["output.dense.weight"], dt), bias=P["output.dense.bias"], out_t=x_t, out_lo=lo_o, rowsum=fold_sums[1],
                     **res_a.gemm_kw())
            return LnResidual(None, fold_sums[1], P["output.LayerNorm.weight"], P["output.LayerNorm.bias"], D, eps, hi=x_t, lo=lo_o), x_t
        ops.gemm(f, WEIGHTS.get(P["output.dense.weight"], dt), bias=P["output.dense.bias"], out32=s_o, out_t=x_t, rowsum=fold_sums[1],
                 **res_a.gemm_kw())
        return LnResidual(s_o, fold_sums[1], P["output.LayerNorm.weight"], P["output.LayerNorm.bias"], D, eps), x_t
    ops.gemm(f, WEIGHTS.get(P["output.dense.weight"], dt), bias=P["output.dense.bias"], out32=s_o,
             **(dict(resid_t=x_t) if t_resid else res_a.gemm_kw()))
    stats_buf = res.stats if (res.dim is None and res.stats is not None) else None
    x_t = _as_act(x_t, M, D, dt, 0)
    return _post_ln(s_o, P["output.LayerNorm.weight"], P["output.LayerNorm.bias"], eps, x_t, stats_buf=stats_buf), x_t


_GRAY_W = {}


def gray_conv_weight(conv_w):
    if conv_w.requires_grad:
        raise NotImplementedError("one-channel input through a TRAINABLE patch embedding: widen the batch instead (src.datasets.segmentation.as_model_input)")
    key = id(conv_w)
    hit = _GRAY_W.get(key)
    sig = (conv_w._version, conv_w.data_ptr(), conv_w.dtype, conv_w.device)
    if hit is None or hit[0] != sig or hit[2]() is not conv_w:
        import weakref
        hit = _GRAY_W[key] = (sig, conv_w.detach().float().sum(dim=1, keepdim=True).contiguous(), weakref.ref(conv_w))
    return hit[1]


class PatchEmbedFn(torch.autograd.Function):

    @staticmethod
    def forward(ctx, images, conv_w, conv_b, cls, pos, patch):
        dt = compute_dtype()
        B, C, H, W = images.shape
        G = (H // patch) * (W // patch)
        D = conv_w.shape[0]
        K = C * patch * patch
# ... 1147 lines not shown
```

### nextgen-uia_amd/uia_hip/ops.py

```python
import ctypes as C
from typing import NamedTuple

import torch

from . import _lib
from ._lib import AttnDesc, GemmDesc, LnLoraDesc, LoraRankDesc, MonaFusedDesc, MonaSpatialDesc, PackDesc, UiaError, WgradGroupDesc, check, lib

_ACT = {None: 0, "none": 0, "gelu": 1, "quick_gelu": 2, "relu": 3}

GEMM_PROFILE = None


EPI_BIAS, EPI_AUX_OUT, EPI_GELU, EPI_DGELU, EPI_RESID, EPI_RESIDT, EPI_OUT32, EPI_OUTT, EPI_RESID_LN, EPI_GENERIC = 1, 2, 4, 8, 16, 32, 64, 128, 256, -1
EPI_QUICK = 2048
EPI_ROWSUM, EPI_LNFOLD = 512, 1024
EPI_RESID_LO, EPI_OUT_LO = 4096, 8192
_SPECIALISED = {EPI_BIAS | EPI_RESID | EPI_OUT32, EPI_BIAS | EPI_RESIDT | EPI_OUT32, EPI_BIAS | EPI_RESID | EPI_RESID_LN | EPI_OUT32, EPI_OUTT, EPI_BIAS | EPI_OUTT, EPI_BIAS | EPI_GELU | EPI_OUTT, EPI_DGELU | EPI_OUTT,
                EPI_BIAS | EPI_GELU | EPI_AUX_OUT | EPI_OUTT,
                EPI_QUICK | EPI_BIAS | EPI_GELU | EPI_OUTT, EPI_QUICK | EPI_DGELU | EPI_OUTT, EPI_QUICK | EPI_BIAS | EPI_GELU | EPI_AUX_OUT | EPI_OUTT,
                EPI_BIAS | EPI_RESID | EPI_OUT32 | EPI_OUTT | EPI_ROWSUM, EPI_BIAS | EPI_RESID | EPI_RESID_LN | EPI_OUT32 | EPI_OUTT | EPI_ROWSUM,
                EPI_BIAS | EPI_OUTT | EPI_LNFOLD, EPI_BIAS | EPI_GELU | EPI_OUTT | EPI_LNFOLD, EPI_BIAS | EPI_GELU | EPI_AUX_OUT | EPI_OUTT | EPI_LNFOLD,
                EPI_QUICK | EPI_BIAS | EPI_GELU | EPI_OUTT | EPI_LNFOLD, EPI_QUICK | EPI_BIAS | EPI_GELU | EPI_AUX_OUT | EPI_OUTT | EPI_LNFOLD,
                EPI_BIAS | EPI_RESID_LO | EPI_RESID_LN | EPI_OUTT | EPI_OUT_LO | EPI_ROWSUM,
                EPI_BIAS | EPI_RESID | EPI_OUTT | EPI_OUT_LO | EPI_ROWSUM, EPI_BIAS | EPI_RESID_LO | EPI_OUT32,
                EPI_BIAS | EPI_RESID | EPI_RESID_LN | EPI_OUTT | EPI_OUT_LO | EPI_ROWSUM, EPI_BIAS | EPI_RESID_LO | EPI_RESID_LN | EPI_OUT32,
                EPI_BIAS | EPI_RESID_LO | EPI_OUT32 | EPI_OUTT | EPI_ROWSUM}

_QUAD_SPECIALISED = _SPECIALISED - {EPI_BIAS | EPI_RESIDT | EPI_OUT32, EPI_BIAS | EPI_RESID | EPI_RESID_LN | EPI_OUT32, EPI_BIAS | EPI_RESID | EPI_RESID_LN | EPI_OUT32 | EPI_OUTT | EPI_ROWSUM,
                                    EPI_BIAS | EPI_RESID | EPI_RESID_LN | EPI_OUTT | EPI_OUT_LO | EPI_ROWSUM, EPI_BIAS | EPI_RESID_LO | EPI_RESID_LN | EPI_OUT32,
                                    EPI_BIAS | EPI_RESID_LO | EPI_OUT32 | EPI_OUTT | EPI_ROWSUM}


def epi_mask_of(d):
    if d.alpha != 1.0 or d.out_group > 0 or d.resid_mod > 0:
        return EPI_GENERIC
    gl = (_ACT["gelu"], _ACT["quick_gelu"])
    if (d.act and d.act not in gl) or (d.dact and d.dact not in gl) or (d.act and d.dact and d.act != d.dact):
        return EPI_GENERIC
    quick = _ACT["quick_gelu"] in (d.act, d.dact)
    m = ((EPI_QUICK if quick else 0) | (EPI_BIAS if d.bias else 0) | (EPI_AUX_OUT if d.aux_out else 0) | (EPI_GELU if d.act else 0) | (EPI_DGELU if d.dact else 0) |
         (EPI_RESID if d.resid else 0) | (EPI_RESIDT if (d.residT and not d.resid_lo8) else 0) | (EPI_OUT32 if d.out32 else 0) | (EPI_OUTT if d.outT else 0) |
         (EPI_RESID_LN if ((d.resid or d.resid_lo8) and d.resid_ln_stats) else 0) | (EPI_ROWSUM if d.rowsum_out else 0) | (EPI_LNFOLD if d.lnfold_sums else 0) |
         (EPI_RESID_LO if d.resid_lo8 else 0) | (EPI_OUT_LO if d.out_lo8 else 0))
    return m


def auto_tile_cfg(M, N, K=None, esz=2, mask=EPI_GENERIC):
    if N <= 64:
        stream64 = N == 64 and M > 2048 and esz == 2 and K is not None and K % 32 == 0 and 64 * (2 * K + 16) <= 160 * 1024
        if stream64 and mask in (EPI_OUTT, EPI_BIAS | EPI_OUTT, EPI_GENERIC):
            return 16
        return 14 if (M > 2048 and esz == 2 and K is not None and K >= 1024) else 4
    if M <= 2048:
        return 21 if (esz == 4 and ((M + 127) // 128) * ((N + 127) // 128) < 64) else 3
    if K is not None and K * esz <= 128:
        return 14
    return 8


RING_CFGS = (8, 9, 10, 12, 13, 14, 24, 25, 26, 27, 28, 29)
PERSIST_STORE_ONLY = False
KBLOCK_W = True
K64_CFG14 = True
TILE_GROUP = {}
SHORT_K_WIDE_HALF_STASH = True
SHORT_K_WIDE_HALF_BYTES = 2048
SHORT_K_WIDE_HALF_N = 3072
HALF_HEIGHT_SHORT_K_ALWAYS = False
HALF_HEIGHT_SHORT_K = True
CHAINS = 1
TAIL_SPLIT = True
TAIL_SIDE_STREAM = True
MONA_PRE_FWD_T = True
MONA_PRE_BWD_DU = True
LN_LORA_DOWN = True
LORA_REGEN_DROP = True
LORA_RANK3 = True
QUAD = False
QUADV = False
RING5 = False
LORA_KEXT = True
TAIL_SPLIT_K = True
_SPLITK_WS = {}
_TRACE_GENERIC = {} if __import__("os").environ.get("UIA_TRACE_GENERIC") else None
_TAIL_SIDE = {}
_NCU = {}


def num_cus(device=None):
# ... 718 lines not shown
    dh = d.dh
    d.dout, d.lddo = _p(dout), dout.stride(-2)
    if is_kb(dq):
        rows, cols, d.dqkv_kb_rows = _kb_dims(dq, "attention dqkv")
        if rows < B * L or cols != 3 * H * dh or dh != 64 or q.dtype != torch.bfloat16 or dk is not None or dv is not None:
            raise UiaError(f"attention dqkv (K-blocked {tuple(dq.t.shape)}) must hold [{B * L}, {3 * H * dh}] bf16 with head dim 64, dk = dv = None")
        part = (H * dh // kb_group(q.dtype)) * d.dqkv_kb_rows * kb_group(q.dtype) * dq.t.element_size()
        d.dq, d.dk, d.dv, d.ld_dqkv = dq.t.data_ptr(), dq.t.data_ptr() + part, dq.t.data_ptr() + 2 * part, cols
    else:
        d.dq, d.dk, d.dv, d.ld_dqkv = _p(dq), _p(dk), _p(dv), dq.stride(-2)
        assert dk.stride(-2) == dq.stride(-2) == dv.stride(-2)
    cfg = ATTN_BWD_CFG if cfg is None else cfg
    if cfg:
        check(lib().uia_attn_bwd_cfg(_stream(), _code(q.dtype), C.byref(d), int(cfg)), "uia_attn_bwd_cfg")
    else:
        check(lib().uia_attn_bwd(_stream(), _code(q.dtype), C.byref(d)), "uia_attn_bwd")


def attn_bwd_cls(q, k, v, out, dout, lse, dq, dk, dv, B, H, L, mask=None, scale=None, rows=False):
    if mask not in (None, "none"):
        raise UiaError(f"attn_bwd_cls: mask {mask!r}: the CLS-query backward takes unmasked attention only")
    d = _attn_desc(q, k, v, out, lse, B, H, L, None, None, scale)
    if d.dh != 64:
        raise UiaError(f"attn_bwd_cls: head dim {d.dh}, only 64 is supported")
    if dout.dim() != 2 or dout.shape[0] != B or dout.shape[1] != H * 64 or dout.stride(1) != 1 or dout.dtype != q.dtype:
        raise UiaError(f"attn_bwd_cls: dout must be [{B}, {H * 64}] {q.dtype} rows (one per sequence), got {tuple(dout.shape)} {dout.dtype}")
    compact = bool(rows)
    if compact and (is_kb(out) or out.dim() != 2 or out.shape[0] != B or out.stride(1) != 1 or out.dtype != q.dtype):
        raise UiaError(f"attn_bwd_cls(rows=True): out must be [{B}, {H * 64}] {q.dtype} rows (one per sequence)")
    if lse is None or lse.dtype != torch.float32 or not lse.is_contiguous() or lse.numel() != (B * H if compact else B * H * L):
        raise UiaError(f"attn_bwd_cls: lse must be a contiguous fp32 [{B}, {H}, {L}] tensor ([{B}, {H}] beside a compact out)")
    d.dout, d.lddo = _p(dout), dout.stride(0)
    if is_kb(dq):
        rows, cols, d.dqkv_kb_rows = _kb_dims(dq, "attention dqkv")
        if rows < B * L or cols != 3 * H * 64 or q.dtype != torch.bfloat16 or dk is not None or dv is not None:
            raise UiaError(f"attention dqkv (K-blocked {tuple(dq.t.shape)}) must hold [{B * L}, {3 * H * 64}] bf16 with head dim 64, dk = dv = None")
        part = (H * 64 // kb_group(q.dtype)) * d.dqkv_kb_rows * kb_group(q.dtype) * dq.t.element_size()
        d.dq, d.dk, d.dv, d.ld_dqkv = dq.t.data_ptr(), dq.t.data_ptr() + part, dq.t.data_ptr() + 2 * part, cols
    else:
        for name, t in (("dq", dq), ("dk", dk), ("dv", dv)):
            if t.dtype != q.dtype or t.dim() != 2 or t.shape[0] < B * L or t.shape[1] != H * 64 or t.stride(1) != 1 or t.stride(0) != dq.stride(0):
                raise UiaError(f"attn_bwd_cls: {name} must be [{B * L}, {H * 64}] {q.dtype} rows sharing one row stride, got {tuple(t.shape)} {t.dtype}")
        d.dq, d.dk, d.dv, d.ld_dqkv = _p(dq), _p(dk), _p(dv), dq.stride(0)
    if compact:
        check(lib().uia_attn_bwd_cls_rows(_stream(), _code(q.dtype), C.byref(d)), "uia_attn_bwd_cls_rows")
    else:
        check(lib().uia_attn_bwd_cls(_stream(), _code(q.dtype), C.byref(d)), "uia_attn_bwd_cls")


def attn_fwd_cls(q, k, v, out, B, H, L, lse=None, mask=None, keylen=None, scale=None):
    if mask not in (None, "none", "keypad"):
        raise UiaError(f"attn_fwd_cls: mask {mask!r}: none or key padding only")
    if is_kb(out) or out.dim() != 2 or out.shape[0] != B or out.shape[1] != H * 64 or out.stride(1) != 1 or out.dtype != q.dtype:
        raise UiaError(f"attn_fwd_cls: out must be [{B}, {H * 64}] {q.dtype} rows (one per sequence)")
    if q.shape[0] < B * L:
        raise UiaError(f"attn_fwd_cls: q / k / v hold {q.shape[0]} rows, {B} sequences of {L} need {B * L}")
    if lse is not None and (lse.dtype != torch.float32 or not lse.is_contiguous() or lse.numel() != B * H):
        raise UiaError(f"attn_fwd_cls: lse must be a contiguous fp32 [{B}, {H}] tensor")
    if mask == "keypad" and (keylen is None or keylen.dtype != torch.int32 or not keylen.is_contiguous() or keylen.numel() != B):
        raise UiaError(f"attn_fwd_cls: key padding needs keylen int32 [{B}]")
    d = _attn_desc(q, k, v, out, lse, B, H, L, mask, keylen if mask == "keypad" else None, scale)
    if d.dh != 64:
        raise UiaError(f"attn_fwd_cls: head dim {d.dh}, only 64 is supported")
    check(lib().uia_attn_fwd_cls(_stream(), _code(q.dtype), C.byref(d)), "uia_attn_fwd_cls")


def rows3_to_f32(hi, lo, stride_rows, dst):
    rows, D = dst.shape
    if dst.dtype != torch.float32 or not dst.is_contiguous() or lo.dtype != torch.int8 or lo.dim() != 2 or lo.stride(1) != 1 or lo.shape[1] != D:
        raise UiaError(f"rows3_to_f32: dst fp32 contiguous [rows, D] and lo int8 [M, D] are required, got {tuple(dst.shape)} {dst.dtype} / {tuple(lo.shape)} {lo.dtype}")
    _require(rows > 0 and stride_rows > 0 and (rows - 1) * stride_rows < lo.shape[0], f"rows3_to_f32: {rows} rows {stride_rows} apart do not fit the {lo.shape[0]} rows of lo")
    if is_kb(hi):
        hrows, hcols, kb_rows = _kb_dims(hi, "rows3_to_f32 hi")
        _require(hi.dtype == torch.bfloat16 and hcols == D and (rows - 1) * stride_rows < hrows, "rows3_to_f32: the K-blocked hi plane must hold bf16 [M, D]")
        hp, ldhi = hi.t.data_ptr(), D
    else:
        _require(hi.dtype == torch.bfloat16 and hi.dim() == 2 and hi.stride(1) == 1 and hi.shape[1] == D and (rows - 1) * stride_rows < hi.shape[0],
                 "rows3_to_f32: the hi plane must hold bf16 [M, D] rows")
        hp, ldhi, kb_rows = hi.data_ptr(), hi.stride(0), 0
    check(lib().uia_rows3_to_f32(_stream(), rows, D, stride_rows, hp, ldhi, kb_rows, _p(lo), lo.stride(0), _p(dst)), "uia_rows3_to_f32")
    return dst


def layernorm_fwd(x, gamma, beta, eps, y_t=None, y32=None, rows=None, ldx=None, stats=None):
    D = gamma.numel()
    rows = x.numel() // D if rows is None else rows
    ldx = D if ldx is None else ldx
    dt = _code(y_t.dtype) if y_t is not None else _lib.F32
    if stats is not None:
        assert stats.dtype == torch.float32 and stats.is_contiguous() and stats.numel() >= 2 * rows
        check(lib().uia_layernorm_fwd_stats(_stream(), dt, rows, D, ldx, _p(x), _p(gamma), _p(beta), eps, _p(y_t), _p(y32), _p(stats)), "uia_layernorm_fwd_stats")
        return
    check(lib().uia_layernorm_fwd(_stream(), dt, rows, D, ldx, _p(x), _p(gamma), _p(beta), eps, _p(y_t), _p(y32)), "uia_layernorm_fwd")


POOL_SLICES = 32


def ln_mean_rows(x, gamma, beta, eps, row0, n, out=None):
    if x.dim() != 3 or x.dtype != torch.float32 or x.stride(-1) != 1 or x.stride(1) != x.shape[2] or x.stride(0) != x.shape[1] * x.shape[2]:
        raise UiaError("ln_mean_rows: x must be a contiguous fp32 [B, L, D] tensor")
    B, L, D = x.shape
    if out is None:
        out = torch.empty(B, D, device=x.device, dtype=torch.float32)
    if out.dtype != torch.float32 or out.stride(-1) != 1 or out.shape[-1] != D or out.shape[0] != B:
        raise UiaError("ln_mean_rows: out must be fp32 [B, D] with unit column stride")
    ws = torch.empty(B * POOL_SLICES * D, device=x.device, dtype=torch.float32)
    check(lib().uia_ln_mean_rows(_stream(), B, L, int(row0), int(n), D, D, _p(x), _p(gamma), _p(beta), float(eps), _p(ws), _p(out), out.stride(0)),
          "uia_ln_mean_rows")
    return out


def layernorm_bwd(dy, x, gamma, eps, dres=None, dx32=None, dx_t=None, rows=None, ldx=None, dx_lo=None):
    D = gamma.numel()
    rows = dy.numel() // D if rows is None else rows
    ldx = D if ldx is None else ldx
    if isinstance(x, tuple) or isinstance(dres, tuple) or dx_lo is not None:
        x_hi, x_lo = x if isinstance(x, tuple) else (None, None)
        r_hi, r_lo = dres if isinstance(dres, tuple) else (None, None)
        x_kb = r_kb = 0
        if is_kb(x_hi):
            kr, kc, x_kb = _kb_dims(x_hi, "layernorm_bwd x hi plane")
            if kr < rows or kc != D:
                raise UiaError(f"layernorm_bwd: K-blocked x hi plane {tuple(x_hi.t.shape)} does not hold [{rows}, {D}]")
            x_hi = x_hi.t
        if is_kb(r_hi):
            kr, kc, r_kb = _kb_dims(r_hi, "layernorm_bwd dres hi plane")
            if kr < rows or kc != D:
                raise UiaError(f"layernorm_bwd: K-blocked dres hi plane {tuple(r_hi.t.shape)} does not hold [{rows}, {D}]")
            r_hi = r_hi.t
        for name, t, dt_ in (("x hi", x_hi, torch.bfloat16), ("x lo", x_lo, torch.int8), ("dres hi", r_hi, torch.bfloat16), ("dres lo", r_lo, torch.int8), ("dx_lo", dx_lo, torch.int8)):
            if t is not None and (t.dtype != dt_ or not t.is_contiguous() or t.numel() < rows * D):
                raise UiaError(f"layernorm_bwd: {name} plane must be a contiguous {dt_} tensor of at least [{rows}, {D}], got {tuple(t.shape)} {t.dtype}")
        check(lib().uia_layernorm_bwd3(_stream(), _code(dy.dtype), rows, D, ldx, _p(dy), None if isinstance(x, tuple) else _p(x), _p(x_hi), _p(x_lo), x_kb, _p(gamma), eps,
                                       None if isinstance(dres, tuple) else _p(dres), _p(r_hi), _p(r_lo), r_kb, _p(dx32), _p(dx_t), _p(dx_lo)), "uia_layernorm_bwd3")
        return
    check(lib().uia_layernorm_bwd(_stream(), _code(dy.dtype), rows, D, ldx, _p(dy), _p(x), _p(gamma), eps, _p(dres), _p(dx32), _p(dx_t)), "uia_layernorm_bwd")


def layernorm_bwd_periodic(dy, x, gamma, eps, dres_rows, period, dx32=None, dx_t=None, dx_lo=None):
    D = gamma.numel()
    M = dy.numel() // D
    nrows = (M + period - 1) // period
    _dense(dres_rows, "layernorm_bwd_periodic: dres_rows", _F32, nrows * D, align=16)
    x_hi, x_lo = x if isinstance(x, tuple) else (None, None)
    x_kb = 0
    if is_kb(x_hi):
        kr, kc, x_kb = _kb_dims(x_hi, "layernorm_bwd_periodic x hi plane")
        if kr < M or kc != D:
            raise UiaError(f"layernorm_bwd_periodic: K-blocked x hi plane {tuple(x_hi.t.shape)} does not hold [{M}, {D}]")
        x_hi = x_hi.t
    for name, t, dt_ in (("dy", dy, dy.dtype), ("x", None if isinstance(x, tuple) else x, torch.float32), ("x hi", x_hi, torch.bfloat16), ("x lo", x_lo, torch.int8),
                         ("dx32", dx32, torch.float32), ("dx_t", dx_t, dy.dtype), ("dx_lo", dx_lo, torch.int8)):
        if t is not None and (t.dtype != dt_ or not t.is_contiguous() or t.numel() < M * D):
            raise UiaError(f"layernorm_bwd_periodic: {name} must be a contiguous {dt_} tensor of at least [{M}, {D}], got {tuple(t.shape)} {t.dtype}")
    check(lib().uia_layernorm_bwd_periodic(_stream(), _code(dy.dtype), M, D, _p(dy), None if isinstance(x, tuple) else _p(x), _p(x_hi), _p(x_lo), x_kb, _p(gamma), eps,
                                           _p(dres_rows), int(period), _p(dx32), _p(dx_t), _p(dx_lo)), "uia_layernorm_bwd_periodic")


def cast(src, dst, scale=1.0):
    _dense(src, "cast: src", _F32, align=16)
    _dense(dst, "cast: dst", _FT, src.numel(), align="v4")
    check(lib().uia_cast(_stream(), _code(dst.dtype), src.numel(), _p(src), _p(dst), scale), "uia_cast")


def transpose_cast(src, dst):
# ... 1012 lines not shown
```

Measured before the change: 6841.

## Fold CLS-only last-layer attention into per-head query projections over raw residual rows

```diff
diff --git a/include/uia_hip.h b/include/uia_hip.h
--- a/include/uia_hip.h
+++ b/include/uia_hip.h
@@ -250,6 +250,32 @@
 int uia_gather_rows(void* stream, int n, int D, const float* src, const int64_t* idx, float* dst);
 int uia_copy_rows(void* stream, int rows, int64_t row_bytes, const void* src, int64_t src_stride_bytes, void* dst);
 int uia_rows3_to_f32(void* stream, int rows, int D, int64_t stride_rows, const void* hi, int64_t ldhi, int64_t hi_kb_rows, const int8_t* lo, int64_t ldlo, float* dst);
+int uia_rows3_from_f32(void* stream, int rows, int D, int64_t stride_rows, const float* src, void* hi, int64_t ldhi, int8_t* lo, int64_t ldlo);
+
+int uia_cls_headwise(void* stream, int contract, int out_dtype, int B, int H, const float* in, const void* W, int64_t ldw, const float* bias, float alpha, void* out);
+typedef struct {
+    int32_t B, H, L, D;
+    const void* x_hi;
+    int64_t ldx, x_kb_rows;
+    const int8_t* x_lo;
+    const void* sums;
+    const float* ln_w;
+    const float* ln_b;
+    float eps;
+    int32_t reserved_;
+    const int32_t* keylen;
+    const float* qt;
+    float* p;
+    float* nbar;
+    const float* g;
+    void* dx_hi;
+    int8_t* dx_lo;
+    float* dqt;
+    float* dn0;
+} uia_cls_fold_desc;
+int uia_attn_cls_fold_fwd(void* stream, const uia_cls_fold_desc* d);
+int uia_attn_cls_fold_bwd(void* stream, const uia_cls_fold_desc* d);
+
 int uia_dropout(void* stream, int dtype, size_t n, const void* src, void* dst, float p, uint64_t seed, int accumulate);
 int uia_colsum(void* stream, int dtype, int M, int N, const void* A, int64_t lda, float* out);
 
diff --git a/nextgen-uia_amd/csrc/capi.cpp b/nextgen-uia_amd/csrc/capi.cpp
--- a/nextgen-uia_amd/csrc/capi.cpp
+++ b/nextgen-uia_amd/csrc/capi.cpp
@@ -104,6 +104,20 @@
 int uia_copy_rows(void* stream, int rows, int64_t row_bytes, const void* src, int64_t src_stride_bytes, void* dst) {
     return uia_copy_rows_launch((hipStream_t)stream, rows, (long)row_bytes, src, (long)src_stride_bytes, dst);
 }
+int uia_rows3_from_f32(void* stream, int rows, int D, int64_t stride_rows, const float* src, void* hi, int64_t ldhi, int8_t* lo, int64_t ldlo) {
+    return uia_rows3_from_f32_launch((hipStream_t)stream, rows, D, (long)stride_rows, src, hi, (long)ldhi, lo, (long)ldlo);
+}
+int uia_cls_headwise(void* stream, int contract, int out_dtype, int B, int H, const float* in, const void* W, int64_t ldw, const float* bias, float alpha, void* out) {
+    return uia_cls_headwise_launch((hipStream_t)stream, contract, out_dtype, B, H, in, W, (long)ldw, bias, alpha, out);
+}
+int uia_attn_cls_fold_fwd(void* stream, const uia_cls_fold_desc* d) {
+    NEED(d, "uia_attn_cls_fold_fwd");
+    return uia_attn_cls_fold_fwd_launch((hipStream_t)stream, *d);
+}
+int uia_attn_cls_fold_bwd(void* stream, const uia_cls_fold_desc* d) {
+    NEED(d, "uia_attn_cls_fold_bwd");
+    return uia_attn_cls_fold_bwd_launch((hipStream_t)stream, *d);
+}
 int uia_cast(void* stream, int dtype, size_t n, const float* src, void* dst, float scale) { return uia_cast_launch((hipStream_t)stream, dtype, n, src, dst, scale); }
 int uia_transpose_cast(void* stream, int dtype, int rows, int cols, const float* src, void* dst) { return uia_transpose_cast_launch((hipStream_t)stream, dtype, rows, cols, src, dst); }
 int uia_pack_weights(void* stream, int dtype, int n, const uia_pack_desc* descs_device, int max_elems) { return uia_pack_weights_launch((hipStream_t)stream, dtype, n, descs_device, max_elems); }
diff --git a/nextgen-uia_amd/csrc/cls_fold.hip b/nextgen-uia_amd/csrc/cls_fold.hip
--- /dev/null
+++ b/nextgen-uia_amd/csrc/cls_fold.hip
@@ -0,0 +1,636 @@
+#include "uia_common.h"
+#include "uia_kernels.h"
+
+namespace {
+
+constexpr int CF_THREADS = 512, CF_WAVES = CF_THREADS / 64;
+constexpr int CF_HMAX = 12, CF_NV = 3;
+constexpr int CF_MAXL = 288, CF_HP = 16;
+constexpr int CF_GROUP = 256, CF_GROUPS = CF_THREADS / CF_GROUP;
+constexpr int CF_DMAX = 64 * CF_HMAX;
+constexpr float CF_ROWSUM_INV = 1.0f / 1073741824.0f;
+enum : int { CF_NORMALISED = 0, CF_SUMS = 1, CF_THREE = 2 };
+
+constexpr int CF_OFF_A = 0, CF_OFF_B = CF_HMAX * CF_DMAX, CF_OFF_S0 = 2 * CF_HMAX * CF_DMAX, CF_OFF_S1 = CF_OFF_S0 + CF_MAXL * CF_HP,
+              CF_OFF_MU = CF_OFF_S1 + CF_MAXL * CF_HP, CF_OFF_RS = CF_OFF_MU + CF_MAXL, CF_OFF_HS = CF_OFF_RS + CF_MAXL, CF_LDS_FLOATS = CF_OFF_HS + 2 * CF_HP;
+constexpr int CF_LDS_BYTES = CF_LDS_FLOATS * 4;
+
+struct CfParams {
+    int B, H, L, D;
+    const bf16_t* x_hi;
+    long ldx, x_kb_rows;
+    const int8_t* x_lo;
+    const long long* sums;
+    const float *ln_w, *ln_b;
+    float eps;
+    const int* keylen;
+    const float* qt;
+    float* p;
+    float* nbar;
+    const float* g;
+    bf16_t* dx_hi;
+    int8_t* dx_lo;
+    float *dqt, *dn0;
+};
+
+__device__ __forceinline__ float dot4(f32x4 a, f32x4 b, float acc) {
+    acc = fmaf(a[0], b[0], acc);
+    acc = fmaf(a[1], b[1], acc);
+    acc = fmaf(a[2], b[2], acc);
+    return fmaf(a[3], b[3], acc);
+}
+
+__device__ __forceinline__ float wave_sum16(const float (&v)[16], int lane) {
+    const bool u5 = lane & 32, u4 = lane & 16, u3 = lane & 8, u2 = lane & 4;
+    float a[8], b[4], c[2];
+#pragma unroll
+    for (int i = 0; i < 8; ++i) a[i] = (u5 ? v[i + 8] : v[i]) + __shfl_xor(u5 ? v[i] : v[i + 8], 32, 64);
+#pragma unroll
+    for (int i = 0; i < 4; ++i) b[i] = (u4 ? a[i + 4] : a[i]) + __shfl_xor(u4 ? a[i] : a[i + 4], 16, 64);
+#pragma unroll
+    for (int i = 0; i < 2; ++i) c[i] = (u3 ? b[i + 2] : b[i]) + __shfl_xor(u3 ? b[i] : b[i + 2], 8, 64);
+    float d = (u2 ? c[1] : c[0]) + __shfl_xor(u2 ? c[0] : c[1], 4, 64);
+    d += uia_dpp_quad_xor1(d);
+    d += uia_dpp_quad_xor2(d);
+    return d;
+}
+
+template <bool THREE>
+struct CfRaw {
+    uint2 h[CF_NV];
+    unsigned l[THREE ? CF_NV : 1];
+};
+
+template <bool THREE>
+__device__ __forceinline__ void cf_fetch(const CfParams& p, size_t row, int lane, int nv, CfRaw<THREE>& r) {
+#pragma unroll
+    for (int k = 0; k < CF_NV; ++k) {
+        const int c4 = lane + 64 * k, col = 4 * c4;
+        r.h[k] = uint2{0u, 0u};
+        if constexpr (THREE) r.l[k] = 0u;
+        if (c4 < nv) {
+            const bf16_t* hp = p.x_kb_rows ? p.x_hi + ((size_t)(col >> 5) * (size_t)p.x_kb_rows + row) * 32 + (col & 31) : p.x_hi + row * (size_t)p.ldx + col;
+            r.h[k] = *(const uint2*)hp;
+            if constexpr (THREE) r.l[k] = *(const unsigned*)(p.x_lo + row * (size_t)p.D + col);
+        }
+    }
+}
+
+template <bool THREE>
+__device__ __forceinline__ f32x4 cf_load4(const CfParams& p, size_t row, int col) {
+    const bf16_t* hp = p.x_kb_rows ? p.x_hi + ((size_t)(col >> 5) * (size_t)p.x_kb_rows + row) * 32 + (col & 31) : p.x_hi + row * (size_t)p.ldx + col;
+    if constexpr (THREE) return three_byte_load4(hp, p.x_lo + row * (size_t)p.D + col);
+    else return load4(hp);
+}
+
+template <int MODE>
+__device__ __forceinline__ float cf_row(const CfParams& p, size_t row, int lane, int nv, const CfRaw<MODE == CF_THREE>& raw, f32x4 (&v)[CF_NV], float& mean) {
+#pragma unroll
+    for (int k = 0; k < CF_NV; ++k) {
+        if constexpr (MODE == CF_THREE) v[k] = three_byte_decode4(raw.h[k], raw.l[k]);
+        else v[k] = f32x4{__builtin_bit_cast(float, raw.h[k].x << 16), __builtin_bit_cast(float, raw.h[k].x & 0xFFFF0000u),
+                          __builtin_bit_cast(float, raw.h[k].y << 16), __builtin_bit_cast(float, raw.h[k].y & 0xFFFF0000u)};
+    }
+    if constexpr (MODE == CF_NORMALISED) {
+        mean = 0.f;
+        return 1.f;
+    }
+    float rstd;
+    if constexpr (MODE == CF_SUMS) {
+        const float inv = 1.0f / (float)p.D;
+        const float s1 = (float)p.sums[2 * row] * CF_ROWSUM_INV, s2 = (float)p.sums[2 * row + 1] * CF_ROWSUM_INV;
+        mean = s1 * inv;
+        rstd = rsqrtf(fmaxf(fmaf(-mean, mean, s2 * inv), 0.0f) + p.eps);
+    } else {
+        float s = 0.f;
+#pragma unroll
+        for (int k = 0; k < CF_NV; ++k) s += v[k][0] + v[k][1] + v[k][2] + v[k][3];
+        mean = wave_sum(s) / p.D;
+    }
+    float q = 0.f;
+#pragma unroll
+    for (int k = 0; k < CF_NV; ++k) {
+        const bool on = lane + 64 * k < nv;
+#pragma unroll
+        for (int e = 0; e < 4; ++e) {
+            const float d = on ? v[k][e] - mean : 0.f;
+            v[k][e] = d;
+            q = fmaf(d, d, q);
+        }
+    }
+    if constexpr (MODE == CF_THREE) rstd = rsqrtf(wave_sum(q) / p.D + p.eps);
+    return rstd;
+}
+
+template <bool THREE, bool SCALE>
+__device__ __forceinline__ void cf_weighted_rows(const CfParams& p, size_t row0, int n, int nv, f32x4 (&acc)[CF_HMAX], const float* cf, const float* mu, const float* rs,
+                                                  float* buf) {
+    const int gi = threadIdx.x / CF_GROUP, tt = threadIdx.x - gi * CF_GROUP, col = 4 * tt, H = p.H, D = p.D;
+    const bool active = tt < nv;
+#pragma unroll
+    for (int h = 0; h < CF_HMAX; ++h) acc[h] = f32x4{0.f, 0.f, 0.f, 0.f};
+    if (active) {
+#pragma unroll 4
+        for (int j = gi; j < n; j += CF_GROUPS) {
+            f32x4 x = cf_load4<THREE>(p, row0 + j, col);
+            const float m = mu[j];
+            const float r = SCALE ? rs[j] : 1.0f;
+#pragma unroll
+            for (int e = 0; e < 4; ++e) x[e] = (x[e] - m) * r;
+            const f32x4* cp = (const f32x4*)(cf + j * CF_HP);
+            const f32x4 c0 = cp[0], c1 = cp[1], c2 = cp[2];
+            const float c[CF_HMAX] = {c0[0], c0[1], c0[2], c0[3], c1[0], c1[1], c1[2], c1[3], c2[0], c2[1], c2[2], c2[3]};
+#pragma unroll
+            for (int h = 0; h < CF_HMAX; ++h)
+                if (h < H) {
+#pragma unroll
+                    for (int e = 0; e < 4; ++e) acc[h][e] = fmaf(c[h], x[e], acc[h][e]);
+                }
+        }
+    }
+    __syncthreads();
+    if (active && gi == 1) {
+#pragma unroll
+        for (int h = 0; h < CF_HMAX; ++h)
+            if (h < H) *(f32x4*)(buf + h * D + col) = acc[h];
+    }
+    __syncthreads();
+    if (active && gi == 0) {
+#pragma unroll
+        for (int h = 0; h < CF_HMAX; ++h)
+            if (h < H) acc[h] += *(const f32x4*)(buf + h * D + col);
+    }
+}
+
+template <int MODE>
+__global__ __launch_bounds__(CF_THREADS) void attn_cls_fold_fwd_kernel(const CfParams p) {
+    extern __shared__ __attribute__((aligned(16))) float lds[];
+    float *qh = lds + CF_OFF_A, *sc = lds + CF_OFF_S0, *mu = lds + CF_OFF_MU, *rs = lds + CF_OFF_RS;
+    const int tid = threadIdx.x, lane = tid & 63, w = tid >> 6;
+    const int b = blockIdx.x, H = p.H, L = p.L, D = p.D, nv = D >> 2;
+    constexpr bool RAW = MODE != CF_NORMALISED;
+    int n = L;
+    if (p.keylen) {
+        n = p.keylen[b];
+        n = n < 1 ? 1 : (n > L ? L : n);
+    }
+    const size_t row0 = (size_t)b * L;
+    for (int i = tid; i < H * nv; i += CF_THREADS) {
+        const int h = i / nv, c4 = i - h * nv;
+        f32x4 q = load4(p.qt + ((size_t)b * H + h) * D + 4 * c4);
+        if (RAW) {
+            const f32x4 lw = load4(p.ln_w + 4 * c4);
+#pragma unroll
+            for (int e = 0; e < 4; ++e) q[e] *= lw[e];
+        }
+        *(f32x4*)(qh + h * D + 4 * c4) = q;
+    }
+    __syncthreads();
+    constexpr bool T3 = MODE == CF_THREE;
+    CfRaw<T3> raw0, raw1;
+    if (w < n) {
+        cf_fetch<T3>(p, row0 + w, lane, nv, raw0);
+        cf_fetch<T3>(p, row0 + (w + CF_WAVES < n ? w + CF_WAVES : w), lane, nv, raw1);
+    }
+    for (int j0 = w; j0 < n; j0 += 2 * CF_WAVES) {
+        const int j1 = j0 + CF_WAVES, jn = j0 + 2 * CF_WAVES;
+        const bool two = j1 < n;
+        f32x4 x0[CF_NV], x1[CF_NV];
+        float m0, m1;
+        const float r0 = cf_row<MODE>(p, row0 + j0, lane, nv, raw0, x0, m0);
+        const float r1 = cf_row<MODE>(p, row0 + (two ? j1 : j0), lane, nv, raw1, x1, m1);
+        if (jn < n) {
+            cf_fetch<T3>(p, row0 + jn, lane, nv, raw0);
+            cf_fetch<T3>(p, row0 + (jn + CF_WAVES < n ? jn + CF_WAVES : jn), lane, nv, raw1);
+        }
+        float d0[16], d1[16];
+#pragma unroll
+        for (int h = 0; h < 16; ++h) {
+            d0[h] = 0.f;
+            d1[h] = 0.f;
+            if (h < CF_HMAX && h < H) {
+#pragma unroll
+                for (int k = 0; k < CF_NV; ++k)
+                    if (lane + 64 * k < nv) {
+                        const f32x4 q = *(const f32x4*)(qh + h * D + 4 * (lane + 64 * k));
+                        d0[h] = dot4(q, x0[k], d0[h]);
+                        d1[h] = dot4(q, x1[k], d1[h]);
+                    }
+            }
+        }
+        const float s0 = wave_sum16(d0, lane) * r0, s1 = wave_sum16(d1, lane) * r1;
+        const int hl = lane >> 2;
+        if ((lane & 3) == 0 && hl < H) {
+            sc[j0 * CF_HP + hl] = s0;
+            if (two) sc[j1 * CF_HP + hl] = s1;
+        }
+        if (lane == 0) {
+            mu[j0] = m0;
+            rs[j0] = r0;
+            if (two) {
+                mu[j1] = m1;
+                rs[j1] = r1;
+            }
+        }
+    }
+    __syncthreads();
+    for (int h = w; h < H; h += CF_WAVES) {
+        constexpr int NP = (CF_MAXL + 63) / 64;
+        float s[NP], m = -INFINITY;
+#pragma unroll
+        for (int t = 0; t < NP; ++t) {
+            const int j = lane + 64 * t;
+            s[t] = j < n ? sc[j * CF_HP + h] : -INFINITY;
+            m = fmaxf(m, s[t]);
+        }
+        m = wave_max(m);
+        float l = 0.f;
+#pragma unroll
+        for (int t = 0; t < NP; ++t) {
+            s[t] = lane + 64 * t < n ? __expf(s[t] - m) : 0.f;
+            l += s[t];
+        }
+        const float inv = 1.0f / wave_sum(l);
+#pragma unroll
+        for (int t = 0; t < NP; ++t) {
+            const int j = lane + 64 * t;
+            if (j < L) {
+                const float pv = s[t] * inv;
+                p.p[((size_t)b * H + h) * L + j] = pv;
+                if (j < n) sc[j * CF_HP + h] = pv * rs[j];
+            }
+        }
+    }
+    __syncthreads();
+    f32x4 acc[CF_HMAX];
+    cf_weighted_rows<MODE == CF_THREE, false>(p, row0, n, nv, acc, sc, mu, rs, qh);
+    if (tid < nv) {
+        const int col = 4 * tid;
+        f32x4 lw = {1.f, 1.f, 1.f, 1.f}, lb = {0.f, 0.f, 0.f, 0.f};
+        if (RAW) {
+            lw = load4(p.ln_w + col);
+            lb = load4(p.ln_b + col);
+        }
+#pragma unroll
+        for (int h = 0; h < CF_HMAX; ++h)
+            if (h < H) {
+                f32x4 o;
+#pragma unroll
+                for (int e = 0; e < 4; ++e) o[e] = fmaf(acc[h][e], lw[e], lb[e]);
+                store4(p.nbar + ((size_t)b * H + h) * D + col, o);
+            }
+    }
+}
+
+__global__ __launch_bounds__(CF_THREADS) void attn_cls_fold_bwd_kernel(const CfParams p) {
+    extern __shared__ __attribute__((aligned(16))) float lds[];
+    float *gw = lds + CF_OFF_A, *qh = lds + CF_OFF_B, *pl = lds + CF_OFF_S0, *ds = lds + CF_OFF_S1, *mu = lds + CF_OFF_MU, *rs = lds + CF_OFF_RS, *hs = lds + CF_OFF_HS,
+          *ssum = lds + CF_OFF_HS + CF_HP;
+    const int tid = threadIdx.x, lane = tid & 63, w = tid >> 6;
+    const int b = blockIdx.x, H = p.H, L = p.L, D = p.D, nv = D >> 2;
+    const size_t row0 = (size_t)b * L, v0 = (size_t)b * H * D;
+    for (int i = tid; i < H * nv; i += CF_THREADS) {
+        const int h = i / nv, c4 = i - h * nv;
+        const f32x4 lw = load4(p.ln_w + 4 * c4);
+        f32x4 g = load4(p.g + v0 + (size_t)h * D + 4 * c4), q = load4(p.qt + v0 + (size_t)h * D + 4 * c4);
+#pragma unroll
+        for (int e = 0; e < 4; ++e) {
+            g[e] *= lw[e];
+            q[e] *= lw[e];
+        }
+        *(f32x4*)(gw + h * D + 4 * c4) = g;
+        *(f32x4*)(qh + h * D + 4 * c4) = q;
+    }
+    for (int i = tid; i < H * L; i += CF_THREADS) {
+        const int h = i / L, j = i - h * L;
+        pl[j * CF_HP + h] = p.p[((size_t)b * H + h) * L + j];
+    }
+    for (int h = w; h < H; h += CF_WAVES) {
+        float a = 0.f;
+#pragma unroll
+        for (int k = 0; k < CF_NV; ++k) {
+            const int c4 = lane + 64 * k;
+            if (c4 < nv) {
+                const f32x4 g = load4(p.g + v0 + (size_t)h * D + 4 * c4), nb = load4(p.nbar + v0 + (size_t)h * D + 4 * c4), lb = load4(p.ln_b + 4 * c4);
+#pragma unroll
+                for (int e = 0; e < 4; ++e) a = fmaf(g[e], lb[e] - nb[e], a);
+            }
+        }
+        a = wave_sum(a);
+        if (lane == 0) hs[h] = a;
+    }
+    __syncthreads();
+    CfRaw<true> raw0, raw1;
+    if (w < L) {
+        cf_fetch<true>(p, row0 + w, lane, nv, raw0);
+        cf_fetch<true>(p, row0 + (w + CF_WAVES < L ? w + CF_WAVES : w), lane, nv, raw1);
+    }
+    for (int j0 = w; j0 < L; j0 += 2 * CF_WAVES) {
+        const int j1 = j0 + CF_WAVES, jn = j0 + 2 * CF_WAVES;
+        const bool two = j1 < L;
+        f32x4 x0[CF_NV], x1[CF_NV], g0[CF_NV], g1[CF_NV];
+        float m0, m1;
+        const float r0 = cf_row<CF_THREE>(p, row0 + j0, lane, nv, raw0, x0, m0);
+        const float r1 = cf_row<CF_THREE>(p, row0 + (two ? j1 : j0), lane, nv, raw1, x1, m1);
+        if (jn < L) {
+            cf_fetch<true>(p, row0 + jn, lane, nv, raw0);
+            cf_fetch<true>(p, row0 + (jn + CF_WAVES < L ? jn + CF_WAVES : jn), lane, nv, raw1);
+        }
+#pragma unroll
+        for (int k = 0; k < CF_NV; ++k) {
+            g0[k] = f32x4{0.f, 0.f, 0.f, 0.f};
+            g1[k] = f32x4{0.f, 0.f, 0.f, 0.f};
+#pragma unroll
+            for (int e = 0; e < 4; ++e) {
+                x0[k][e] *= r0;
+                x1[k][e] *= r1;
+            }
+        }
+        float t0[16], t1[16];
+#pragma unroll
+        for (int h = 0; h < 16; ++h) {
+            t0[h] = 0.f;
+            t1[h] = 0.f;
+            if (h < CF_HMAX && h < H) {
+#pragma unroll
+                for (int k = 0; k < CF_NV; ++k)
+                    if (lane + 64 * k < nv) {
+                        const f32x4 gv = *(const f32x4*)(gw + h * D + 4 * (lane + 64 * k));
+                        t0[h] = dot4(gv, x0[k], t0[h]);
+                        t1[h] = dot4(gv, x1[k], t1[h]);
+                    }
+            }
+        }
+        const float s0 = wave_sum16(t0, lane), s1 = wave_sum16(t1, lane);
+        const int hl = lane >> 2;
+        if ((lane & 3) == 0 && hl < H) {
+            const float off = hs[hl];
+            ds[j0 * CF_HP + hl] = pl[j0 * CF_HP + hl] * (s0 + off);
+            if (two) ds[j1 * CF_HP + hl] = pl[j1 * CF_HP + hl] * (s1 + off);
+        }
+        const f32x4 *pa = (const f32x4*)(pl + j0 * CF_HP), *pb = (const f32x4*)(pl + (two ? j1 : j0) * CF_HP);
+        const f32x4 *da = (const f32x4*)(ds + j0 * CF_HP), *db = (const f32x4*)(ds + (two ? j1 : j0) * CF_HP);
+        const f32x4 pa0 = pa[0], pa1 = pa[1], pa2 = pa[2], pb0 = pb[0], pb1 = pb[1], pb2 = pb[2];
+        const f32x4 da0 = da[0], da1 = da[1], da2 = da[2], db0 = db[0], db1 = db[1], db2 = db[2];
+        const float P0[CF_HMAX] = {pa0[0], pa0[1], pa0[2], pa0[3], pa1[0], pa1[1], pa1[2], pa1[3], pa2[0], pa2[1], pa2[2], pa2[3]};
+        const float P1[CF_HMAX] = {pb0[0], pb0[1], pb0[2], pb0[3], pb1[0], pb1[1], pb1[2], pb1[3], pb2[0], pb2[1], pb2[2], pb2[3]};
+        const float D0[CF_HMAX] = {da0[0], da0[1], da0[2], da0[3], da1[0], da1[1], da1[2], da1[3], da2[0], da2[1], da2[2], da2[3]};
+        const float D1[CF_HMAX] = {db0[0], db0[1], db0[2], db0[3], db1[0], db1[1], db1[2], db1[3], db2[0], db2[1], db2[2], db2[3]};
+#pragma unroll
+        for (int h = 0; h < CF_HMAX; ++h)
+            if (h < H) {
+#pragma unroll
+                for (int k = 0; k < CF_NV; ++k)
+                    if (lane + 64 * k < nv) {
+                        const f32x4 gv = *(const f32x4*)(gw + h * D + 4 * (lane + 64 * k));
+                        const f32x4 q = *(const f32x4*)(qh + h * D + 4 * (lane + 64 * k));
+#pragma unroll
+                        for (int e = 0; e < 4; ++e) {
+                            g0[k][e] = fmaf(P0[h], gv[e], fmaf(D0[h], q[e], g0[k][e]));
+                            g1[k][e] = fmaf(P1[h], gv[e], fmaf(D1[h], q[e], g1[k][e]));
+                        }
+                    }
+            }
+        if (lane == 0) {
+            mu[j0] = m0;
+            rs[j0] = r0;
+            if (two) {
+                mu[j1] = m1;
+                rs[j1] = r1;
+            }
+        }
+        float sg0 = 0.f, sx0 = 0.f, sg1 = 0.f, sx1 = 0.f;
+#pragma unroll
+        for (int k = 0; k < CF_NV; ++k)
+#pragma unroll
+            for (int e = 0; e < 4; ++e) {
+                sg0 += g0[k][e];
+                sx0 = fmaf(g0[k][e], x0[k][e], sx0);
+                sg1 += g1[k][e];
+                sx1 = fmaf(g1[k][e], x1[k][e], sx1);
+            }
+        const float mg0 = wave_sum(sg0) / D, mx0 = wave_sum(sx0) / D, mg1 = wave_sum(sg1) / D, mx1 = wave_sum(sx1) / D;
+#pragma unroll
+        for (int k = 0; k < CF_NV; ++k) {
+            const int c4 = lane + 64 * k;
+            if (c4 < nv) {
+                f32x4 o0, o1;
+#pragma unroll
+                for (int e = 0; e < 4; ++e) {
+                    o0[e] = r0 * (g0[k][e] - mg0 - x0[k][e] * mx0);
+                    o1[e] = r1 * (g1[k][e] - mg1 - x1[k][e] * mx1);
+                }
+                if (j0 > 0) three_byte_store4(p.dx_hi + (row0 + j0) * D + 4 * c4, p.dx_lo + (row0 + j0) * D + 4 * c4, o0);
+                if (two) three_byte_store4(p.dx_hi + (row0 + j1) * D + 4 * c4, p.dx_lo + (row0 + j1) * D + 4 * c4, o1);
+            }
+        }
+    }
+    __syncthreads();
+    for (int h = w; h < H; h += CF_WAVES) {
+        float a = 0.f;
+        for (int j = lane; j < L; j += 64) a += ds[j * CF_HP + h];
+        a = wave_sum(a);
+        if (lane == 0) ssum[h] = a;
+    }
+    if (tid >= CF_THREADS - CF_GROUP && tid - (CF_THREADS - CF_GROUP) < nv) {
+        const int col = 4 * (tid - (CF_THREADS - CF_GROUP));
+        f32x4 o = {0.f, 0.f, 0.f, 0.f};
+        for (int h = 0; h < H; ++h) {
+            const f32x4 g = load4(p.g + v0 + (size_t)h * D + col), q = load4(p.qt + v0 + (size_t)h * D + col);
+            const float p0 = pl[h], d0 = ds[h];
+#pragma unroll
+            for (int e = 0; e < 4; ++e) o[e] = fmaf(p0, g[e], fmaf(d0, q[e], o[e]));
+        }
+        store4(p.dn0 + (size_t)b * D + col, o);
+    }
+    __syncthreads();
+    f32x4 acc[CF_HMAX];
+    cf_weighted_rows<true, true>(p, row0, L, nv, acc, ds, mu, rs, gw);
+    if (tid < nv) {
+        const int col = 4 * tid;
+        const f32x4 lw = load4(p.ln_w + col), lb = load4(p.ln_b + col);
+#pragma unroll
+        for (int h = 0; h < CF_HMAX; ++h)
+            if (h < H) {
+                const float sh = ssum[h];
+                f32x4 o;
+#pragma unroll
+                for (int e = 0; e < 4; ++e) o[e] = fmaf(acc[h][e], lw[e], lb[e] * sh);
+                store4(p.dqt + v0 + (size_t)h * D + col, o);
+            }
+    }
+}
+
+constexpr int HW_ROWS = 8;
+
+__global__ __launch_bounds__(256) void cls_headwise_expand_kernel(int B, int H, int D, const float* __restrict__ in, const bf16_t* __restrict__ W, long ldw, float alpha,
+                                                                  float* __restrict__ out) {
+    __shared__ float xin[HW_ROWS][64];
+    const int tid = threadIdx.x, h = blockIdx.x, b0 = blockIdx.y * HW_ROWS, nv = D >> 2;
+    for (int i = tid; i < HW_ROWS * 64; i += 256) {
+        const int bi = i >> 6, d = i & 63;
+        xin[bi][d] = b0 + bi < B ? in[(size_t)(b0 + bi) * D + h * 64 + d] : 0.f;
+    }
+    __syncthreads();
+    if (tid >= nv) return;
+    const int col = 4 * tid;
+    f32x4 acc[HW_ROWS];
+#pragma unroll
+    for (int bi = 0; bi < HW_ROWS; ++bi) acc[bi] = f32x4{0.f, 0.f, 0.f, 0.f};
+#pragma unroll 16
+    for (int d = 0; d < 64; ++d) {
+        const f32x4 wv = load4(W + (size_t)(h * 64 + d) * ldw + col);
+#pragma unroll
+        for (int bi = 0; bi < HW_ROWS; ++bi) {
+            const float x = xin[bi][d];
+#pragma unroll
+            for (int e = 0; e < 4; ++e) acc[bi][e] = fmaf(x, wv[e], acc[bi][e]);
+        }
+    }
+#pragma unroll
+    for (int bi = 0; bi < HW_ROWS; ++bi)
+        if (b0 + bi < B) {
+            f32x4 o;
+#pragma unroll
+            for (int e = 0; e < 4; ++e) o[e] = acc[bi][e] * alpha;
+            store4(out + ((size_t)(b0 + bi) * H + h) * D + col, o);
+        }
+}
+
+template <typename TO>
+__global__ __launch_bounds__(256) void cls_headwise_contract_kernel(int B, int H, int D, const float* __restrict__ in, const bf16_t* __restrict__ W, long ldw,
+                                                                    const float* __restrict__ bias, float alpha, TO* __restrict__ out, long ldo) {
+    __shared__ float res[HW_ROWS][64];
+    const int tid = threadIdx.x, lane = tid & 63, w = tid >> 6, h = blockIdx.x, b0 = blockIdx.y * HW_ROWS, nv = D >> 2;
+    f32x4 x[HW_ROWS][CF_NV];
+#pragma unroll
+    for (int bi = 0; bi < HW_ROWS; ++bi)
+#pragma unroll
+        for (int k = 0; k < CF_NV; ++k) {
+            const int c4 = lane + 64 * k;
+            x[bi][k] = (c4 < nv && b0 + bi < B) ? load4(in + ((size_t)(b0 + bi) * H + h) * D + 4 * c4) : f32x4{0.f, 0.f, 0.f, 0.f};
+        }
+    for (int d = w; d < 64; d += 8) {
+        f32x4 wa[CF_NV], wb[CF_NV];
+#pragma unroll
+        for (int k = 0; k < CF_NV; ++k) {
+            const int c4 = lane + 64 * k;
+            wa[k] = c4 < nv ? load4(W + (size_t)(h * 64 + d) * ldw + 4 * c4) : f32x4{0.f, 0.f, 0.f, 0.f};
+            wb[k] = c4 < nv ? load4(W + (size_t)(h * 64 + d + 4) * ldw + 4 * c4) : f32x4{0.f, 0.f, 0.f, 0.f};
+        }
+        float s[16];
+#pragma unroll
+        for (int bi = 0; bi < HW_ROWS; ++bi) {
+            s[bi] = 0.f;
+            s[HW_ROWS + bi] = 0.f;
+#pragma unroll
+            for (int k = 0; k < CF_NV; ++k) {
+                s[bi] = dot4(x[bi][k], wa[k], s[bi]);
+                s[HW_ROWS + bi] = dot4(x[bi][k], wb[k], s[HW_ROWS + bi]);
+            }
+        }
+        const float t = wave_sum16(s, lane);
+        const int i = lane >> 2;
+        if ((lane & 3) == 0) res[i & (HW_ROWS - 1)][d + 4 * (i >> 3)] = t;
+    }
+    __syncthreads();
+    for (int i = tid; i < HW_ROWS * 64; i += 256) {
+        const int bi = i >> 6, d = i & 63;
+        if (b0 + bi < B) out[(size_t)(b0 + bi) * ldo + h * 64 + d] = from_f32<TO>(fmaf(alpha, res[bi][d], bias ? bias[h * 64 + d] : 0.f));
+    }
+}
+
+__global__ __launch_bounds__(256) void rows3_from_kernel(int rows, int D, long stride, const float* __restrict__ src, bf16_t* __restrict__ hi, long ldhi, int8_t* __restrict__ lo,
+                                                         long ldlo) {
+    const long i = (long)blockIdx.x * 256 + threadIdx.x;
+    const int nv = D >> 2;
+    if (i >= (long)rows * nv) return;
+    const long r = i / nv, row = r * stride;
+    const int col = 4 * (int)(i - r * nv);
+    three_byte_store4(hi + row * ldhi + col, lo + row * ldlo + col, load4(src + r * D + col));
+}
+
+int cf_check(const char* who, const uia_cls_fold_desc& d, bool bwd) {
+    UIA_CHECK_ARG(d.B > 0 && d.H > 0 && d.H <= CF_HMAX && d.L > 0 && d.L <= CF_MAXL, "%s: B=%d H=%d L=%d outside the supported range (H <= 12, L <= 288)", who, d.B, d.H, d.L);
+    UIA_CHECK_ARG(d.D == 64 * d.H, "%s: D=%d is not 64 per head (H=%d)", who, d.D, d.H);
+    UIA_CHECK_ARG(d.x_hi && d.qt && d.p && d.nbar, "%s: null tensor", who);
+    UIA_CHECK_ARG(d.x_kb_rows ? d.x_kb_rows >= (int64_t)d.B * d.L : (d.ldx >= d.D && d.ldx % 4 == 0),
+                  "%s: input rows closer than D (or not whole 8-byte units), or a K-blocked plane of fewer than B*L rows", who);
+    UIA_CHECK_ARG(((uintptr_t)d.x_hi % 8) == 0 && ((uintptr_t)d.x_lo % 4) == 0 && ((uintptr_t)d.sums % 16) == 0 && ((uintptr_t)d.keylen % 4) == 0 && ((uintptr_t)d.p % 4) == 0 &&
+                  (((uintptr_t)d.qt | (uintptr_t)d.nbar | (uintptr_t)d.ln_w | (uintptr_t)d.ln_b | (uintptr_t)d.g | (uintptr_t)d.dqt | (uintptr_t)d.dn0) % 16) == 0 &&
+                  ((uintptr_t)d.dx_hi % 8) == 0 && ((uintptr_t)d.dx_lo % 4) == 0, "%s: alignment", who);
+    UIA_CHECK_ARG(d.eps >= 0.f && d.eps < 1.0f, "%s: eps=%g", who, (double)d.eps);
+    if (bwd) {
+        UIA_CHECK_ARG(d.x_lo && !d.sums && d.ln_w && d.ln_b && !d.keylen, "%s: the backward reads the three-byte input (x_lo) with the LayerNorm weight and bias, unmasked", who);
+        UIA_CHECK_ARG(d.g && d.dx_hi && d.dx_lo && d.dqt && d.dn0, "%s: null tensor", who);
+    } else {
+        UIA_CHECK_ARG(!(d.x_lo && d.sums), "%s: a three-byte input recomputes its statistics; row sums beside low bytes are refused", who);
+        UIA_CHECK_ARG((d.x_lo || d.sums) ? (d.ln_w && d.ln_b) : (!d.ln_w && !d.ln_b), "%s: raw rows (sums or low bytes) come with the LayerNorm weight and bias, normalised rows without", who);
+    }
+    return 0;
+}
+
+CfParams cf_params(const uia_cls_fold_desc& d) {
+    CfParams p;
+    p.B = d.B; p.H = d.H; p.L = d.L; p.D = d.D;
+    p.x_hi = (const bf16_t*)d.x_hi; p.ldx = (long)d.ldx; p.x_kb_rows = (long)d.x_kb_rows; p.x_lo = d.x_lo;
+    p.sums = (const long long*)d.sums; p.ln_w = d.ln_w; p.ln_b = d.ln_b; p.eps = d.eps; p.keylen = d.keylen;
+    p.qt = d.qt; p.p = d.p; p.nbar = d.nbar; p.g = d.g; p.dx_hi = (bf16_t*)d.dx_hi; p.dx_lo = d.dx_lo; p.dqt = d.dqt; p.dn0 = d.dn0;
+    return p;
+}
+
+}
+
+int uia_attn_cls_fold_fwd_launch(hipStream_t stream, const uia_cls_fold_desc& d) {
+    if (cf_check("uia_attn_cls_fold_fwd", d, false)) return -1;
+    const CfParams p = cf_params(d);
+    const dim3 grid(d.B), block(CF_THREADS);
+    static UiaDevOnce once0, once1, once2;
+    if (d.x_lo) {
+        UIA_ENSURE_LDS_ATTR(once2, attn_cls_fold_fwd_kernel<CF_THREE>, CF_LDS_BYTES);
+        hipLaunchKernelGGL(attn_cls_fold_fwd_kernel<CF_THREE>, grid, block, CF_LDS_BYTES, stream, p);
+    } else if (d.sums) {
+        UIA_ENSURE_LDS_ATTR(once1, attn_cls_fold_fwd_kernel<CF_SUMS>, CF_LDS_BYTES);
+        hipLaunchKernelGGL(attn_cls_fold_fwd_kernel<CF_SUMS>, grid, block, CF_LDS_BYTES, stream, p);
+    } else {
+        UIA_ENSURE_LDS_ATTR(once0, attn_cls_fold_fwd_kernel<CF_NORMALISED>, CF_LDS_BYTES);
+        hipLaunchKernelGGL(attn_cls_fold_fwd_kernel<CF_NORMALISED>, grid, block, CF_LDS_BYTES, stream, p);
+    }
+    UIA_CHECK_LAUNCH();
+    return 0;
+}
+
+int uia_attn_cls_fold_bwd_launch(hipStream_t stream, const uia_cls_fold_desc& d) {
+    if (cf_check("uia_attn_cls_fold_bwd", d, true)) return -1;
+    const CfParams p = cf_params(d);
+    static UiaDevOnce once;
+    UIA_ENSURE_LDS_ATTR(once, attn_cls_fold_bwd_kernel, CF_LDS_BYTES);
+    hipLaunchKernelGGL(attn_cls_fold_bwd_kernel, dim3(d.B), dim3(CF_THREADS), CF_LDS_BYTES, stream, p);
+    UIA_CHECK_LAUNCH();
+    return 0;
+}
+
+int uia_cls_headwise_launch(hipStream_t stream, int contract, int out_dtype, int B, int H, const float* in, const void* W, long ldw, const float* bias, float alpha, void* out) {
+    UIA_CHECK_ARG(B > 0 && H > 0 && H <= CF_HMAX, "uia_cls_headwise: B=%d H=%d outside the supported range (H <= 12)", B, H);
+    UIA_CHECK_ARG(out_dtype == UIA_BF16 || out_dtype == UIA_F32, "uia_cls_headwise: bad output dtype %d", out_dtype);
+    UIA_CHECK_ARG(contract || (out_dtype == UIA_F32 && !bias), "uia_cls_headwise: the expanding form writes fp32 [B, H, 64*H] and takes no bias");
+    const int D = 64 * H;
+    UIA_CHECK_ARG(in && W && out && ldw >= D && ldw % 4 == 0, "uia_cls_headwise: null tensor, or weight rows closer than 64*H (or not whole 8-byte units)");
+    UIA_CHECK_ARG(((uintptr_t)in % 16) == 0 && ((uintptr_t)W % 8) == 0 && ((uintptr_t)out % 16) == 0 && ((uintptr_t)bias % 4) == 0, "uia_cls_headwise: alignment");
+    const dim3 grid(H, (B + HW_ROWS - 1) / HW_ROWS), block(256);
+    if (!contract) hipLaunchKernelGGL(cls_headwise_expand_kernel, grid, block, 0, stream, B, H, D, in, (const bf16_t*)W, ldw, alpha, (float*)out);
+    else if (out_dtype == UIA_BF16) hipLaunchKernelGGL(cls_headwise_contract_kernel<bf16_t>, grid, block, 0, stream, B, H, D, in, (const bf16_t*)W, ldw, bias, alpha, (bf16_t*)out, (long)D);
+    else hipLaunchKernelGGL(cls_headwise_contract_kernel<float>, grid, block, 0, stream, B, H, D, in, (const bf16_t*)W, ldw, bias, alpha, (float*)out, (long)D);
+    UIA_CHECK_LAUNCH();
+    return 0;
+}
+
+int uia_rows3_from_f32_launch(hipStream_t stream, int rows, int D, long stride_rows, const float* src, void* hi, long ldhi, int8_t* lo, long ldlo) {
+    UIA_CHECK_ARG(rows > 0 && D > 0 && D % 4 == 0 && stride_rows > 0 && (long)rows * D <= 0x7FFFFFFFL, "uia_rows3_from_f32: %d rows of %d elements, %ld apart", rows, D, stride_rows);
+    UIA_CHECK_ARG(src && hi && lo && ldhi >= D && ldlo >= D && ldhi % 4 == 0 && ldlo % 4 == 0, "uia_rows3_from_f32: null tensor, or plane rows closer than D (or not whole 4-element units)");
+    UIA_CHECK_ARG(((uintptr_t)src % 16) == 0 && ((uintptr_t)hi % 8) == 0 && ((uintptr_t)lo % 4) == 0, "uia_rows3_from_f32: alignment");
+    const long total = (long)rows * (D / 4);
+    hipLaunchKernelGGL(rows3_from_kernel, dim3((unsigned)((total + 255) / 256)), dim3(256), 0, stream, rows, D, stride_rows, src, (bf16_t*)hi, ldhi, lo, ldlo);
+    UIA_CHECK_LAUNCH();
+    return 0;
+}
diff --git a/nextgen-uia_amd/csrc/uia_kernels.h b/nextgen-uia_amd/csrc/uia_kernels.h
--- a/nextgen-uia_amd/csrc/uia_kernels.h
+++ b/nextgen-uia_amd/csrc/uia_kernels.h
@@ -28,6 +28,10 @@
 int uia_mona_cls_bwd_launch(hipStream_t stream, int dtype, int B, int ntok, const void* dd, const void* t, long ldt, void* dt, float p_drop, uint64_t seed,
                             const uint8_t* keep_mask);
 int uia_copy_rows_launch(hipStream_t stream, int rows, long row_bytes, const void* src, long src_stride_bytes, void* dst);
+int uia_attn_cls_fold_fwd_launch(hipStream_t stream, const uia_cls_fold_desc& d);
+int uia_attn_cls_fold_bwd_launch(hipStream_t stream, const uia_cls_fold_desc& d);
+int uia_cls_headwise_launch(hipStream_t stream, int contract, int out_dtype, int B, int H, const float* in, const void* W, long ldw, const float* bias, float alpha, void* out);
+int uia_rows3_from_f32_launch(hipStream_t stream, int rows, int D, long stride_rows, const float* src, void* hi, long ldhi, int8_t* lo, long ldlo);
 int uia_lora_rank_update_launch(hipStream_t stream, int dtype, const uia_lora_rank_desc& p);
 int uia_ln_lora_down_launch(hipStream_t stream, int dtype, const uia_ln_lora_desc& p);
 int uia_cast_launch(hipStream_t stream, int dtype, size_t n, const float* src, void* dst, float scale);
diff --git a/nextgen-uia_amd/uia_hip/_lib.py b/nextgen-uia_amd/uia_hip/_lib.py
--- a/nextgen-uia_amd/uia_hip/_lib.py
+++ b/nextgen-uia_amd/uia_hip/_lib.py
@@ -39,6 +39,11 @@
                 ("B", i32), ("H", i32), ("L", i32), ("dh", i32), ("mask_kind", i32), ("scale", f32),
                 ("dout", vp), ("lddo", i64), ("dq", vp), ("dk", vp), ("dv", vp), ("ld_dqkv", i64), ("cu_seqlens", vp),
                 ("out_kb_rows", i64), ("dqkv_kb_rows", i64)]
+
+
+class ClsFoldDesc(C.Structure):
+    _fields_ = [("B", i32), ("H", i32), ("L", i32), ("D", i32), ("x_hi", vp), ("ldx", i64), ("x_kb_rows", i64), ("x_lo", vp), ("sums", vp), ("ln_w", vp), ("ln_b", vp),
+                ("eps", f32), ("reserved_", i32), ("keylen", vp), ("qt", vp), ("p", vp), ("nbar", vp), ("g", vp), ("dx_hi", vp), ("dx_lo", vp), ("dqt", vp), ("dn0", vp)]
 
 
 class MonaSpatialDesc(C.Structure):
@@ -188,6 +193,10 @@
     "uia_mona_cls_fwd": (C.c_int, [vp, C.c_int, C.c_int, C.c_int, vp, i64, vp, f32, C.c_uint64, vp]),
     "uia_rows3_to_f32": (C.c_int, [vp, C.c_int, C.c_int, i64, vp, i64, i64, vp, i64, vp]),
     "uia_layernorm_bwd_periodic": (C.c_int, [vp, C.c_int, C.c_int, C.c_int, vp, vp, vp, vp, i64, vp, f32, vp, C.c_int, vp, vp, vp]),
+    "uia_rows3_from_f32": (C.c_int, [vp, C.c_int, C.c_int, i64, vp, vp, i64, vp, i64]),
+    "uia_cls_headwise": (C.c_int, [vp, C.c_int, C.c_int, C.c_int, C.c_int, vp, vp, i64, vp, f32, vp]),
+    "uia_attn_cls_fold_fwd": (C.c_int, [vp, C.POINTER(ClsFoldDesc)]),
+    "uia_attn_cls_fold_bwd": (C.c_int, [vp, C.POINTER(ClsFoldDesc)]),
 }
 
 _lib = None
diff --git a/nextgen-uia_amd/uia_hip/functional.py b/nextgen-uia_amd/uia_hip/functional.py
--- a/nextgen-uia_amd/uia_hip/functional.py
+++ b/nextgen-uia_amd/uia_hip/functional.py
@@ -247,6 +247,23 @@
             bias = bias.contiguous()
         out = (ops.PackedW(wf), colsum, bias)
         self._c[key] = (vers, weakref.ref(w), out, weakref.ref(ln_w))
+        return out
+
+    def get_cls_fold(self, w, b, dt):
+        key = (id(w), dt, "clsfold")
+        vers = (w._version, -1 if b is None else b._version, w.device)
+        hit = self._c.get(key)
+        if hit is not None and hit[0] == vers and hit[1]() is w:
+            return hit[2]
+        with torch.no_grad():
+            D = w.shape[1]
+            w32 = w.detach().float()
+            wt = w32[D:].to(dt).contiguous()
+            b32 = b.detach().float().contiguous() if b is not None else torch.zeros(3 * D, device=w.device)
+            wq, wq_t = w32[:D].contiguous(), w32[:D].t().contiguous()
+            bq, bv = b32[:D].contiguous(), b32[2 * D:].contiguous()
+        out = dict(wq=ops.PackedW(wq), wq_t=ops.PackedW(wq_t), bq=bq, wk=wt[:D], wv=wt[D:], bv=bv)
+        self._c[key] = (vers, weakref.ref(w), out)
         return out
 
     def get_cat(self, ws, dt, transpose=False):
@@ -581,6 +598,53 @@
     return MonaFn.apply(x_bnd, variant, tuple(hw), pd, keep_mask, names, direct, *params)
 
 
+def set_cls_attention_fold(flag):
+    _STATE["cls_attn_fold"] = bool(flag)
+
+
+def cls_attention_fold_enabled():
+    return _STATE.get("cls_attn_fold", True)
+
+
+def _cls_fold_ok(dt, M, L, heads, D):
+    return (cls_attention_fold_enabled() and dt == torch.bfloat16 and ln_fold_enabled(dt, M) and 1 < L <= ops.CLS_FOLD_MAX_L and heads <= ops.CLS_FOLD_MAX_H
+            and D == 64 * heads)
+
+
+def _cls_fold_fwd(h_cls, x_hi, W, B, heads, L, dt, x_lo=None, sums=None, ln=None, keylen=None):
+    D = 64 * heads
+    q = torch.empty(B, D, device=h_cls.device, dtype=torch.float32)
+    ops.gemm(h_cls, W["wq"], bias=W["bq"], out32=q)
+    qt = torch.empty(B, heads, D, device=h_cls.device, dtype=torch.float32)
+    ops.cls_headwise(q, W["wk"], qt, alpha=0.125)
+    p = torch.empty(B, heads, L, device=h_cls.device, dtype=torch.float32)
+    nbar = torch.empty(B, heads, D, device=h_cls.device, dtype=torch.float32)
+    ops.attn_cls_fold_fwd(x_hi, qt, p, nbar, B, heads, L, x_lo=x_lo, sums=sums, ln=ln, keylen=keylen)
+    a = torch.empty(B, D, device=h_cls.device, dtype=dt)
+    ops.cls_headwise(nbar, W["wv"], a, contract=True, bias=W["bv"])
+    return a, (p, qt, nbar)
+
+
+def _cls_fold_bwd(W, ln, B, heads, L, dt, xin, p_att, qt, nbar, x_cls, da, dx1):
+    D = 64 * heads
+    M, dev = B * L, x_cls.device
+    g = torch.empty(B, heads, D, device=dev, dtype=torch.float32)
+    ops.cls_headwise(da, W["wv"], g)
+    dx_t = torch.empty(M, D, device=dev, dtype=dt)
+    dlo = torch.empty(M, D, device=dev, dtype=torch.int8)
+    dqt = torch.empty(B, heads, D, device=dev, dtype=torch.float32)
+    dn0 = torch.empty(B, D, device=dev, dtype=torch.float32)
+    ops.attn_cls_fold_bwd(xin.hi, xin.lo, ln, p_att, g, qt, nbar, dx_t, dlo, dqt, dn0, B, heads, L)
+    dq = torch.empty(B, D, device=dev, dtype=torch.float32)
+    ops.cls_headwise(dqt, W["wk"], dq, contract=True, alpha=0.125)
+    dh0 = torch.empty(B, D, device=dev, dtype=torch.float32)
+    ops.gemm(dq, W["wq_t"], resid=dn0, out32=dh0)
+    dx0 = torch.empty(B, D, device=dev, dtype=torch.float32)
+    ops.layernorm_bwd(dh0, x_cls, ln[0], ln[2], dres=dx1, dx32=dx0)
+    ops.rows3_from_f32(dx0, L, dx_t, dlo)
+    return dx_t, dlo
+
+
 class BlockSpec:
 
     def __init__(self, heads, eps, act, ln1, qkv, proj, ln2, fc1, fc2, mask=None, publish_out=False):
@@ -614,6 +678,9 @@
             rows = (x3.hi, x3.sums)
         else:
             rows = take_rows(x, dt) if fold else None
+        cls_path = handoff.take_last_block_cls() and spec.mask is None and 1 < N <= ATTN_SINGLE_PASS_MAX and D == 64 * spec.heads and like.is_cuda
+        if cls_path and x3 is not None and _cls_fold_ok(dt, M, N, spec.heads, D) and (not train or _g3_partner_feeds(x)):
+            return VitBlockFn._forward_cls(ctx, x, x3, None, spec, (B, N, D), dt, train)
         qkv = _empty((M, 3 * D), dt, like)
         if rows is not None:
             wq, cq, bq = WEIGHTS.get_lnfold(spec.qkv[0], spec.qkv[1], spec.ln1[0], spec.ln1[1], dt)
@@ -626,7 +693,7 @@
             h1 = _empty((M, D), dt, x)
             ops.layernorm_fwd(x2d, spec.ln1[0], spec.ln1[1], spec.eps, y_t=h1)
             ops.gemm(h1, WEIGHTS.get(spec.qkv[0], dt), bias=spec.qkv[1], out_t=qkv)
-        if handoff.take_last_block_cls() and spec.mask is None and 1 < N <= ATTN_SINGLE_PASS_MAX and D == 64 * spec.heads and like.is_cuda:
+        if cls_path:
             return VitBlockFn._forward_cls(ctx, x, x3, qkv, spec, (B, N, D), dt, train)
         if N > ATTN_SINGLE_PASS_MAX:
             a = _empty((M, D), dt, like)
@@ -675,15 +742,22 @@
     @staticmethod
     def _forward_cls(ctx, x, x3, qkv, spec, shape, dt, train):
         B, N, D = shape
-        like = qkv
-        a = _empty((B, D), dt, like)
-        lse = torch.empty(B, spec.heads, device=like.device, dtype=torch.float32) if train else None
-        ops.attn_fwd_cls(qkv[:, :D], qkv[:, D:2 * D], qkv[:, 2 * D:], a, B, spec.heads, N, lse=lse)
+        fold = qkv is None
+        like = x3.lo if fold else qkv
         x_cls = torch.empty(B, D, device=like.device, dtype=torch.float32)
         if x3 is not None:
             ops.rows3_to_f32(x3.hi, x3.lo, N, x_cls)
         else:
             ops.copy_rows(x.view(B * N, D), N, x_cls)
+        if fold:
+            h_cls = torch.empty(B, D, device=like.device, dtype=torch.float32)
+            ops.layernorm_fwd(x_cls, spec.ln1[0], spec.ln1[1], spec.eps, y32=h_cls)
+            a, kept = _cls_fold_fwd(h_cls, x3.hi, WEIGHTS.get_cls_fold(spec.qkv[0], spec.qkv[1], dt), B, spec.heads, N, dt, x_lo=x3.lo,
+                                    ln=(spec.ln1[0], spec.ln1[1], spec.eps))
+        else:
+            a = _empty((B, D), dt, like)
+            lse = torch.empty(B, spec.heads, device=like.device, dtype=torch.float32) if train else None
+            ops.attn_fwd_cls(qkv[:, :D], qkv[:, D:2 * D], qkv[:, 2 * D:], a, B, spec.heads, N, lse=lse)
         x1 = torch.empty(B, D, device=like.device, dtype=torch.float32)
         M = B * N
         wp = WEIGHTS.get(spec.proj[0], dt)
@@ -698,25 +772,33 @@
         x2 = torch.empty(B, 1, D, device=like.device, dtype=torch.float32)
         ops.gemm(f, w2, bias=spec.fc2[1], resid=x1, out32=x2.view(B, D), tile_cfg=_rows_tile_cfg(M, w2, like, dt, out32=True, resid=True))
         if train:
-            saved, ctx.layout = handoff.save_layout(x3.resid3 if x3 is not None else x, qkv, a, lse, x1, pre)
+            if fold:
+                saved, ctx.layout = handoff.save_layout(x3.resid3, kept[0], kept[1], kept[2], x_cls, x1, pre)
+            else:
+                saved, ctx.layout = handoff.save_layout(x3.resid3 if x3 is not None else x, qkv, a, lse, x1, pre)
             ctx.save_for_backward(*saved)
             ctx.xshape = (B, N, D)
             ctx.spec = spec
             ctx.g3_out = dt == torch.bfloat16 and _g3_partner_feeds(x)
             ctx.cls_ok = False
             ctx.cls_fwd = True
+            ctx.attn_fold = fold
         handoff.cls_rows_out(True)
         return x2
 
     @staticmethod
     def backward_cls(ctx, cg):
         compact = getattr(ctx, "cls_fwd", False)
-        xin, qkv, a, lse, x1, pre = handoff.restore_layout(ctx.saved_tensors, ctx.layout)
+        fold = getattr(ctx, "attn_fold", False)
+        if fold:
+            xin, p_att, qt, nbar, x_cls, x1, pre = handoff.restore_layout(ctx.saved_tensors, ctx.layout)
+        else:
+            xin, qkv, a, lse, x1, pre = handoff.restore_layout(ctx.saved_tensors, ctx.layout)
         x3_in = isinstance(xin, Resid3)
         x = xin.lo if x3_in else xin
         spec = ctx.spec
         B, N, D = ctx.xshape
-        M, dt = B * N, qkv.dtype
+        M, dt = B * N, pre.dtype
         F = pre.shape[1]
         dy = cg.rows32
         dy_t = dy if dt == torch.float32 else (cg.rows_t if cg.rows_t is not None else t_copy_of(dy, dt))
@@ -729,6 +811,12 @@
         dx1 = _empty((B, D), torch.float32, x)
         dx1_t = _empty((B, D), dt, x) if dt != torch.float32 else dx1
         ops.layernorm_bwd(dh, x1_cls, spec.ln2[0], spec.eps, dres=dy, dx32=dx1, dx_t=dx1_t if dt != torch.float32 else None)
+        if fold:
+            da = torch.empty(B, D, device=x.device, dtype=torch.float32)
+            ops.gemm(dx1_t, WEIGHTS.get(spec.proj[0], dt, transpose=True), out32=da)
+            dx_t, dlo = _cls_fold_bwd(WEIGHTS.get_cls_fold(spec.qkv[0], spec.qkv[1], dt), (spec.ln1[0], spec.ln1[1], spec.eps), B, spec.heads, N, dt, xin, p_att, qt, nbar,
+                                      x_cls, da, dx1)
+            return publish_grad3((B, N, D), x.device, dx_t, dlo), None
         da = dh
         ops.gemm(dx1_t, WEIGHTS.get(spec.proj[0], dt, transpose=True), out_t=da)
         dqkv = _attn_act(M, 3 * D, dt, x, D)
@@ -869,10 +957,22 @@
     return cu_seqlens is None and D == 64 * heads and 1 < L <= 288 and x_t.is_cuda and not (x_t.dtype != torch.float32 and _STATE.get("text_resid_t", False))
 
 
-def _post_ln_layer_cls(res, qkv, L, B, heads, P, keylen, eps, D, dt):
-    a = _empty((B, D), dt, qkv)
-    ops.attn_fwd_cls(qkv[:, :D], qkv[:, D:2 * D], qkv[:, 2 * D:], a, B, heads, L, mask="keypad", keylen=keylen)
+def _post_ln_layer_cls(res, qkv, L, B, heads, P, keylen, eps, D, dt, x_t=None):
     r = _res_cls_rows(res, L, B, D, eps)
+    if qkv is None:
+        qkv = r
+        h_cls = r
+        W = WEIGHTS.get_cls_fold(P["_qkv_raw"][0], P["_qkv_raw"][1], dt)
+        ln = (res.w, res.b, res.eps if res.eps is not None else eps)
+        if res.lo is not None:
+            a, _ = _cls_fold_fwd(h_cls, x_t, W, B, heads, L, dt, x_lo=res.lo, ln=ln, keylen=keylen)
+        elif res.dim is not None:
+            a, _ = _cls_fold_fwd(h_cls, x_t, W, B, heads, L, dt, sums=res.stats, ln=ln, keylen=keylen)
+        else:
+            a, _ = _cls_fold_fwd(h_cls, x_t, W, B, heads, L, dt, keylen=keylen)
+    else:
+        a = _empty((B, D), dt, qkv)
+        ops.attn_fwd_cls(qkv[:, :D], qkv[:, D:2 * D], qkv[:, 2 * D:], a, B, heads, L, mask="keypad", keylen=keylen)
     s_a = torch.empty(B, D, device=qkv.device, dtype=torch.float32)
     M = B * L
     wo = WEIGHTS.get(P["attention.output.dense.weight"], dt)
@@ -894,6 +994,8 @@
     dt = x_t.dtype
     t_resid = dt != torch.float32 and _STATE.get("text_resid_t", False)
     fold = fold_sums is not None and ln_fold_enabled(dt, M) and not t_resid
+    if cls_only and _cls_fold_ok(dt, M, L, heads, D) and "_qkv_raw" in P:
+        return _post_ln_layer_cls(res, None, L, B, heads, P, keylen, eps, D, dt, x_t=x_t)
     qkv = _empty((M, 3 * D), dt, x_t)
     if res.dim is not None:
         wq, cq, bq = WEIGHTS.get_lnfold(P["_qkv_raw"][0], P["_qkv_raw"][1], res.w, res.b, dt)
diff --git a/nextgen-uia_amd/uia_hip/ops.py b/nextgen-uia_amd/uia_hip/ops.py
--- a/nextgen-uia_amd/uia_hip/ops.py
+++ b/nextgen-uia_amd/uia_hip/ops.py
@@ -4,7 +4,7 @@
 import torch
 
 from . import _lib
-from ._lib import AttnDesc, GemmDesc, LnLoraDesc, LoraRankDesc, MonaFusedDesc, MonaSpatialDesc, PackDesc, UiaError, WgradGroupDesc, check, lib
+from ._lib import AttnDesc, ClsFoldDesc, GemmDesc, LnLoraDesc, LoraRankDesc, MonaFusedDesc, MonaSpatialDesc, PackDesc, UiaError, WgradGroupDesc, check, lib
 
 _ACT = {None: 0, "none": 0, "gelu": 1, "quick_gelu": 2, "relu": 3}
 
@@ -889,6 +889,81 @@
     return dst
 
 
+def rows3_from_f32(src, stride_rows, hi, lo):
+    rows, D = src.shape
+    _dense(src, "rows3_from_f32: src", _F32, rows * D, align=16)
+    for name, t, dt_ in (("hi", hi, torch.bfloat16), ("lo", lo, torch.int8)):
+        if t.dtype != dt_ or t.dim() != 2 or t.stride(1) != 1 or t.shape[1] != D or (rows - 1) * stride_rows >= t.shape[0]:
+            raise UiaError(f"rows3_from_f32: {name} must hold {dt_} [M, {D}] rows with M > {(rows - 1) * stride_rows}, got {tuple(t.shape)} {t.dtype}")
+    check(lib().uia_rows3_from_f32(_stream(), rows, D, stride_rows, _p(src), _p(hi), hi.stride(0), _p(lo), lo.stride(0)), "uia_rows3_from_f32")
+
+
+CLS_FOLD_MAX_L, CLS_FOLD_MAX_H = 288, 12
+
+
+def cls_headwise(inp, w, out, contract=False, bias=None, alpha=1.0):
+    D = w.shape[1]
+    H = D // 64
+    B = inp.shape[0]
+    if w.dtype != torch.bfloat16 or w.dim() != 2 or w.shape[0] != D or D != 64 * H or w.stride(1) != 1:
+        raise UiaError(f"cls_headwise: w must be a bf16 [64·H, 64·H] slice with unit column stride, got {tuple(w.shape)} {w.dtype}")
+    _dense(inp, "cls_headwise: inp", _F32, B * H * D if contract else B * D, align=16)
+    _dense(out, "cls_headwise: out", _FT if contract else _F32, B * D if contract else B * H * D, align=16)
+    if bias is not None:
+        _dense(bias, "cls_headwise: bias", _F32, D)
+    check(lib().uia_cls_headwise(_stream(), int(contract), _code(out.dtype), B, H, _p(inp), _p(w), w.stride(0), _p(bias), float(alpha), _p(out)), "uia_cls_headwise")
+    return out
+
+
+def _cls_fold_desc(who, x_hi, x_lo, B, H, L):
+    d = ClsFoldDesc()
+    D = 64 * H
+    d.B, d.H, d.L, d.D = B, H, L, D
+    if is_kb(x_hi):
+        hrows, hcols, kb_rows = _kb_dims(x_hi, f"{who} x_hi")
+        _require(x_hi.dtype == torch.bfloat16 and hcols == D and hrows >= B * L, f"{who}: the K-blocked input plane must hold bf16 [{B * L}, {D}]")
+        d.x_hi, d.ldx, d.x_kb_rows = x_hi.t.data_ptr(), D, kb_rows
+    else:
+        _require(x_hi.dtype == torch.bfloat16 and x_hi.dim() == 2 and x_hi.stride(1) == 1 and x_hi.shape[1] == D and x_hi.shape[0] >= B * L,
+                 f"{who}: the input plane must hold bf16 [{B * L}, {D}] rows")
+        d.x_hi, d.ldx, d.x_kb_rows = x_hi.data_ptr(), x_hi.stride(0), 0
+    if x_lo is not None:
+        _dense(x_lo, f"{who}: x_lo", (torch.int8,), B * L * D, align=4)
+        d.x_lo = _p(x_lo)
+    return d, D
+
+
+def attn_cls_fold_fwd(x_hi, qt, p, nbar, B, H, L, x_lo=None, sums=None, ln=None, keylen=None):
+    d, D = _cls_fold_desc("attn_cls_fold_fwd", x_hi, x_lo, B, H, L)
+    _dense(qt, "attn_cls_fold_fwd: qt", _F32, B * H * D, align=16)
+    _dense(p, "attn_cls_fold_fwd: p", _F32, B * H * L)
+    _dense(nbar, "attn_cls_fold_fwd: nbar", _F32, B * H * D, align=16)
+    if sums is not None:
+        _dense(sums, "attn_cls_fold_fwd: sums", (torch.int64,), 2 * B * L, align=16)
+        d.sums = _p(sums)
+    if ln is not None:
+        _dense(ln[0], "attn_cls_fold_fwd: LayerNorm weight", _F32, D, align=16)
+        _dense(ln[1], "attn_cls_fold_fwd: LayerNorm bias", _F32, D, align=16)
+        d.ln_w, d.ln_b, d.eps = _p(ln[0]), _p(ln[1]), float(ln[2])
+    if keylen is not None:
+        _dense(keylen, "attn_cls_fold_fwd: keylen", (torch.int32,), B)
+        d.keylen = _p(keylen)
+    d.qt, d.p, d.nbar = _p(qt), _p(p), _p(nbar)
+    check(lib().uia_attn_cls_fold_fwd(_stream(), C.byref(d)), "uia_attn_cls_fold_fwd")
+
+
+def attn_cls_fold_bwd(x_hi, x_lo, ln, p, g, qt, nbar, dx_hi, dx_lo, dqt, dn0, B, H, L):
+    d, D = _cls_fold_desc("attn_cls_fold_bwd", x_hi, x_lo, B, H, L)
+    for name, t, n in (("p", p, B * H * L), ("g", g, B * H * D), ("qt", qt, B * H * D), ("nbar", nbar, B * H * D), ("dqt", dqt, B * H * D), ("dn0", dn0, B * D),
+                       ("LayerNorm weight", ln[0], D), ("LayerNorm bias", ln[1], D)):
+        _dense(t, f"attn_cls_fold_bwd: {name}", _F32, n, align=4 if name == "p" else 16)
+    _dense(dx_hi, "attn_cls_fold_bwd: dx_hi", (torch.bfloat16,), B * L * D, align=8)
+    _dense(dx_lo, "attn_cls_fold_bwd: dx_lo", (torch.int8,), B * L * D, align=4)
+    d.ln_w, d.ln_b, d.eps = _p(ln[0]), _p(ln[1]), float(ln[2])
+    d.qt, d.p, d.nbar, d.g, d.dx_hi, d.dx_lo, d.dqt, d.dn0 = _p(qt), _p(p), _p(nbar), _p(g), _p(dx_hi), _p(dx_lo), _p(dqt), _p(dn0)
+    check(lib().uia_attn_cls_fold_bwd(_stream(), C.byref(d)), "uia_attn_cls_fold_bwd")
+
+
 def layernorm_fwd(x, gamma, beta, eps, y_t=None, y32=None, rows=None, ldx=None, stats=None):
     D = gamma.numel()
     rows = x.numel() // D if rows is None else rows
```

Result: no change. 6884, median of 6 (+0.6%).
